# jianshu93/lash

Hardware: AMD Instinct MI355X
Metric: k-mers/s sketched (hmh, k=16) (higher is better)
Workload: dtype u64; 1 GPU; 12500 synthetic 5000000-bp genomes per GPU, -a hmh -k 16, seed 42, ASCII records resident in HBM -> sketch images in HBM (lash_sketch_batch_device: filter_out_n + k-mers + xxh3 + registers + images); genomes_per_gpu=12500, genome_length=5000000, records_per_gpu=12500, dirty=none, algo=hmh, k=16, p=0, layout=default

## Files before the change

### include/lash_gfx950.h

```cpp
#ifndef LASH_GFX950_H
#define LASH_GFX950_H
#include <stddef.h>
#include <stdint.h>

#ifdef __cplusplus
extern "C" {
#endif

#define LASH_ABI_VERSION 5

#define LASH_OK       0
#define LASH_EINVAL  (-1)
#define LASH_ENODEV  (-2)
#define LASH_EHIP    (-3)
#define LASH_ENOMEM  (-4)
#define LASH_ERANGE  (-6)
#define LASH_EFORMAT (-7)
#define LASH_ELIMIT  (-5)

#define LASH_HMH 0
#define LASH_HLL 1
#define LASH_ULL 2

#define LASH_F_HMH_X_LOW   1u
#define LASH_F_ACCUMULATE  2u
#define LASH_F_AMINO       8u
#define LASH_F_NO_DIRECT   4u

#define LASH_F_STREAM_ONLY 16u

#define LASH_F_NO_SOLE     32u

typedef struct lash_ctx lash_ctx;
typedef struct lash_packed lash_packed;

typedef struct {
    int32_t  algo;
    int32_t  k;
    int32_t  p;
    uint32_t flags;
    uint64_t seed;
} lash_params;

typedef struct {
    uint8_t base_code[4];
    uint8_t kmer_lsb_first;
    uint8_t hmh_x_low;
    uint8_t hmh_reg_be;
    uint8_t hll_bucket_high;
    char    hmh_header[8];
    char    hll_header[8];
    char    ull_header[8];
    uint8_t fastq_skip_bad;
    uint8_t aa_code_zero_based;
    uint8_t reserved[6];
} lash_layout;

typedef struct {
    float    pack_ms;
    float    sketch_ms;
    float    finalize_ms;
    uint32_t calls;
    uint32_t sketch_launches;
    uint32_t sketch_workgroups;
    uint32_t direct_launches;
    uint64_t kmers;
    uint64_t bases_last;
    uint64_t packed_bytes;
    float    direct_ms;
    uint32_t defer_launches;
    uint32_t sole_launches;
} lash_timing;

int         lash_abi_version(void);
int         lash_device_count(void);
const char *lash_strerror(int code);
int         lash_ctx_create(lash_ctx **out, int device);
void        lash_ctx_destroy(lash_ctx *ctx);
int         lash_ctx_set_stream(lash_ctx *ctx, void *hip_stream);
int         lash_ctx_synchronize(lash_ctx *ctx);
const char *lash_ctx_last_error(lash_ctx *ctx);
int         lash_ctx_enable_timing(lash_ctx *ctx, int on);
int         lash_ctx_get_timing(lash_ctx *ctx, lash_timing *out);

void       *lash_host_alloc_pinned(size_t bytes);
void        lash_host_free_pinned(void *p);

int         lash_params_check(const lash_params *prm);
size_t      lash_sketch_image_bytes(int algo, int p);

void        lash_layout_default(lash_layout *out);
int         lash_layout_check(const lash_layout *lay);
int         lash_layout_parse(const char *spec, lash_layout *out);
size_t      lash_layout_header_bytes(const lash_layout *lay, int algo);
size_t      lash_layout_image_bytes(const lash_layout *lay, int algo, int p);
int         lash_ctx_set_layout(lash_ctx *ctx, const lash_layout *lay);
int         lash_ctx_get_layout(lash_ctx *ctx, lash_layout *out);

int lash_sketch_batch(lash_ctx *ctx, const lash_params *prm,
                      const uint8_t *seq, const uint64_t *rec_off, uint64_t n_rec,
                      const uint64_t *genome_rec_off, uint32_t n_genomes, uint8_t *out_images);

int lash_sketch_batch_async(lash_ctx *ctx, const lash_params *prm,
                            const uint8_t *seq, const uint64_t *rec_off, uint64_t n_rec,
                            const uint64_t *genome_rec_off, uint32_t n_genomes, uint8_t *out_images);

int lash_sketch_batch_device(lash_ctx *ctx, const lash_params *prm,
                             const uint8_t *d_seq, const uint64_t *d_rec_off, uint64_t n_rec,
                             const uint64_t *genome_rec_off, const uint64_t *genome_byte_off,
                             uint32_t n_genomes, uint8_t *d_out_images);

#define LASH_FMT_FASTA 1
#define LASH_FMT_FASTQ 2
int lash_sketch_files_raw(lash_ctx *ctx, const lash_params *prm, const uint8_t *raw, const uint64_t *file_off,
                          const uint8_t *file_fmt, uint32_t n_files, uint8_t *out_images);
int lash_sketch_files_raw_device(lash_ctx *ctx, const lash_params *prm, const uint8_t *d_raw, const uint64_t *file_off,
                                 const uint8_t *file_fmt, uint32_t n_files, uint8_t *d_out_images);
uint32_t lash_ctx_format_errors(lash_ctx *ctx, uint32_t *file_index, uint32_t cap);

typedef struct lash_rec_index lash_rec_index;
int      lash_fasta_index(lash_ctx *ctx, const uint8_t *raw, const uint64_t *file_off, uint32_t n_files, lash_rec_index **out);
int      lash_fasta_index_device(lash_ctx *ctx, const uint8_t *d_raw, const uint64_t *file_off, uint32_t n_files, lash_rec_index **out);
uint64_t lash_rec_index_n_records(const lash_rec_index *index);
int      lash_rec_index_start(lash_ctx *ctx, const lash_rec_index *index, uint64_t *out);
int      lash_rec_index_id_len(lash_ctx *ctx, const lash_rec_index *index, uint32_t *out);
int      lash_rec_index_file(lash_ctx *ctx, const lash_rec_index *index, uint32_t *out);
void     lash_rec_index_free(lash_ctx *ctx, lash_rec_index *index);
int      lash_sketch_records_raw(lash_ctx *ctx, const lash_params *prm, const uint8_t *raw, const uint64_t *file_off, uint32_t n_files,
                                 const lash_rec_index *index, uint64_t r0, uint64_t r1, uint8_t *out_images);

typedef struct lash_win_index lash_win_index;
int      lash_fasta_windows(lash_ctx *ctx, const uint8_t *raw, const uint64_t *file_off, uint32_t n_files, const lash_rec_index *index,
                            uint64_t window, lash_win_index **out);
int      lash_fasta_windows_device(lash_ctx *ctx, const uint8_t *d_raw, const uint64_t *file_off, uint32_t n_files, const lash_rec_index *index,
                                   uint64_t window, lash_win_index **out);
uint64_t lash_win_index_n_windows(const lash_win_index *windows);
uint64_t lash_win_index_bytes(const lash_win_index *windows);
const uint8_t *lash_win_index_buffer_device(const lash_win_index *windows);
int      lash_win_index_record(lash_ctx *ctx, const lash_win_index *windows, uint64_t *out);
int      lash_win_index_begin(lash_ctx *ctx, const lash_win_index *windows, uint64_t *out);
int      lash_win_index_length(lash_ctx *ctx, const lash_win_index *windows, uint64_t *out);
int      lash_win_index_offset(lash_ctx *ctx, const lash_win_index *windows, uint64_t *out);
int      lash_sketch_windows_raw(lash_ctx *ctx, const lash_params *prm, const lash_win_index *windows, uint64_t w0, uint64_t w1,
                                 uint8_t *out_images);
void     lash_win_index_free(lash_ctx *ctx, lash_win_index *windows);

typedef struct lash_tr_index lash_tr_index;
int      lash_fasta_translate(lash_ctx *ctx, const uint8_t *raw, const uint64_t *file_off, uint32_t n_files, const lash_rec_index *index,
                              lash_tr_index **out);
int      lash_fasta_translate_device(lash_ctx *ctx, const uint8_t *d_raw, const uint64_t *file_off, uint32_t n_files, const lash_rec_index *index,
                                     lash_tr_index **out);
uint64_t lash_tr_index_n_segments(const lash_tr_index *translated);
uint64_t lash_tr_index_bytes(const lash_tr_index *translated);
const uint8_t *lash_tr_index_buffer_device(const lash_tr_index *translated);
// ... 166 lines not shown
```

### lash_amd/_lib.py

```python
import ctypes as C
import os

PKG = os.path.dirname(os.path.abspath(__file__))
LIB_PATH = os.environ.get("LASH_GFX950_LIB") or os.path.join(PKG, "liblash_gfx950.so")

OK, EINVAL, ENODEV, EHIP, ENOMEM, ELIMIT, ERANGE, EFORMAT = 0, -1, -2, -3, -4, -5, -6, -7
HMH, HLL, ULL = 0, 1, 2
F_HMH_X_LOW, F_ACCUMULATE, F_NO_DIRECT, F_AMINO, F_STREAM_ONLY, F_NO_SOLE = 1, 2, 4, 8, 16, 32
FMT_FASTA, FMT_FASTQ = 1, 2
MEASURE_JACCARD, MEASURE_CONTAIN_QUERY, MEASURE_CONTAIN_REFERENCE = 0, 1, 2
ABI_VERSION = 5


class Params(C.Structure):
    _fields_ = [("algo", C.c_int32), ("k", C.c_int32), ("p", C.c_int32), ("flags", C.c_uint32), ("seed", C.c_uint64)]


class Layout(C.Structure):
    _fields_ = [("base_code", C.c_uint8 * 4), ("kmer_lsb_first", C.c_uint8), ("hmh_x_low", C.c_uint8),
                ("hmh_reg_be", C.c_uint8), ("hll_bucket_high", C.c_uint8),
                ("hmh_header", C.c_char * 8), ("hll_header", C.c_char * 8), ("ull_header", C.c_char * 8),
                ("fastq_skip_bad", C.c_uint8), ("aa_code_zero_based", C.c_uint8), ("reserved", C.c_uint8 * 6)]


class Timing(C.Structure):
    _fields_ = [("pack_ms", C.c_float), ("sketch_ms", C.c_float), ("finalize_ms", C.c_float), ("calls", C.c_uint32),
                ("sketch_launches", C.c_uint32), ("sketch_workgroups", C.c_uint32), ("direct_launches", C.c_uint32),
                ("kmers", C.c_uint64), ("bases_last", C.c_uint64), ("packed_bytes", C.c_uint64),
                ("direct_ms", C.c_float), ("defer_launches", C.c_uint32), ("sole_launches", C.c_uint32)]


class ClusterStats(C.Structure):
    _fields_ = [("pairs", C.c_uint64), ("pruned", C.c_uint64), ("joined_on_device", C.c_uint64), ("sent_to_host", C.c_uint64),
                ("clusters", C.c_uint64)]


class DerepStats(C.Structure):
    _fields_ = [("pairs", C.c_uint64), ("pruned_not_rep", C.c_uint64), ("pruned_after_hit", C.c_uint64), ("sent_to_host", C.c_uint64),
                ("evaluated", C.c_uint64), ("representatives", C.c_uint64)]


class TreeMerge(C.Structure):
    _fields_ = [("a", C.c_uint32), ("b", C.c_uint32), ("height", C.c_double), ("size", C.c_uint32)]


class TreeStats(C.Structure):
    _fields_ = [("steps", C.c_uint64), ("rescanned_rows", C.c_uint64), ("bytes", C.c_uint64)]


class NjJoin(C.Structure):
    _fields_ = [("a", C.c_uint32), ("b", C.c_uint32), ("len_a", C.c_double), ("len_b", C.c_double)]


LINKAGE_AVERAGE, LINKAGE_SINGLE, LINKAGE_COMPLETE = 0, 1, 2

_vp, _u64, _u32, _int = C.c_void_p, C.c_uint64, C.c_uint32, C.c_int
_PP = C.POINTER(Params)
_LP = C.POINTER(Layout)

PROTOTYPES = {
    "lash_abi_version": (_int, []),
    "lash_device_count": (_int, []),
    "lash_strerror": (C.c_char_p, [_int]),
    "lash_ctx_create": (_int, [C.POINTER(_vp), _int]),
    "lash_ctx_destroy": (None, [_vp]),
    "lash_ctx_set_stream": (_int, [_vp, _vp]),
    "lash_ctx_synchronize": (_int, [_vp]),
    "lash_ctx_last_error": (C.c_char_p, [_vp]),
    "lash_ctx_enable_timing": (_int, [_vp, _int]),
    "lash_ctx_get_timing": (_int, [_vp, C.POINTER(Timing)]),
    "lash_host_alloc_pinned": (_vp, [C.c_size_t]),
    "lash_host_free_pinned": (None, [_vp]),
    "lash_params_check": (_int, [_PP]),
    "lash_sketch_image_bytes": (C.c_size_t, [_int, _int]),
    "lash_layout_default": (None, [_LP]),
    "lash_layout_check": (_int, [_LP]),
    "lash_layout_parse": (_int, [C.c_char_p, _LP]),
    "lash_layout_header_bytes": (C.c_size_t, [_LP, _int]),
    "lash_layout_image_bytes": (C.c_size_t, [_LP, _int, _int]),
    "lash_ctx_set_layout": (_int, [_vp, _LP]),
    "lash_ctx_get_layout": (_int, [_vp, _LP]),
    "lash_sketch_batch": (_int, [_vp, _PP, _vp, _vp, _u64, _vp, _u32, _vp]),
    "lash_sketch_batch_async": (_int, [_vp, _PP, _vp, _vp, _u64, _vp, _u32, _vp]),
    "lash_sketch_batch_device": (_int, [_vp, _PP, _vp, _vp, _u64, _vp, _vp, _u32, _vp]),
    "lash_sketch_files_raw": (_int, [_vp, _PP, _vp, _vp, _vp, _u32, _vp]),
    "lash_sketch_files_raw_device": (_int, [_vp, _PP, _vp, _vp, _vp, _u32, _vp]),
    "lash_ctx_format_errors": (_u32, [_vp, _vp, _u32]),
    "lash_kmer_filter_create": (_int, [_vp, _u32, _vp, C.POINTER(_vp)]),
    "lash_kmer_filter_count_raw": (_int, [_vp, _PP, _vp, _vp, _vp, _u32, _vp]),
    "lash_kmer_filter_counts": (_int, [_vp, _vp, _u32, _vp]),
    "lash_sketch_files_raw_filtered": (_int, [_vp, _PP, _vp, _vp, _vp, _u32, _vp, _u32, _vp]),
    "lash_kmer_filter_free": (None, [_vp, _vp]),
    "lash_fasta_index": (_int, [_vp, _vp, _vp, _u32, C.POINTER(_vp)]),
    "lash_fasta_index_device": (_int, [_vp, _vp, _vp, _u32, C.POINTER(_vp)]),
    "lash_rec_index_n_records": (_u64, [_vp]),
    "lash_rec_index_start": (_int, [_vp, _vp, _vp]),
    "lash_rec_index_id_len": (_int, [_vp, _vp, _vp]),
    "lash_rec_index_file": (_int, [_vp, _vp, _vp]),
    "lash_rec_index_free": (None, [_vp, _vp]),
    "lash_sketch_records_raw": (_int, [_vp, _PP, _vp, _vp, _u32, _vp, _u64, _u64, _vp]),
    "lash_fasta_windows": (_int, [_vp, _vp, _vp, _u32, _vp, _u64, C.POINTER(_vp)]),
    "lash_fasta_windows_device": (_int, [_vp, _vp, _vp, _u32, _vp, _u64, C.POINTER(_vp)]),
    "lash_win_index_n_windows": (_u64, [_vp]),
    "lash_win_index_bytes": (_u64, [_vp]),
    "lash_win_index_buffer_device": (_vp, [_vp]),
    "lash_win_index_record": (_int, [_vp, _vp, _vp]),
    "lash_win_index_begin": (_int, [_vp, _vp, _vp]),
    "lash_win_index_length": (_int, [_vp, _vp, _vp]),
    "lash_win_index_offset": (_int, [_vp, _vp, _vp]),
    "lash_sketch_windows_raw": (_int, [_vp, _PP, _vp, _u64, _u64, _vp]),
    "lash_win_index_free": (None, [_vp, _vp]),
    "lash_fasta_translate": (_int, [_vp, _vp, _vp, _u32, _vp, C.POINTER(_vp)]),
# ... 106 lines not shown
```

### lash_amd/csrc/lash_api.hip

```cpp
#include "lash_ctx.h"
#include "lash_internal.h"



namespace lashi {

size_t parse_fastx_strict(const uint8_t *d, size_t n, std::vector<uint8_t> *seq, std::vector<uint64_t> *rec_off, bool skip_bad,
                                 std::vector<std::pair<size_t, size_t>> *bad)
{
    auto line_end = [&](size_t p) { const void *q = memchr(d + p, '\n', n - p); return q ? (size_t)((const uint8_t *)q - d) : n; };
    size_t i = 0;
    if (n && d[0] == '>') {
        while (i < n) {
            i = line_end(i);
            if (i < n) ++i;
            while (i < n && d[i] != '>') {
                size_t e = line_end(i), stop = e;
                while (stop > i && d[stop - 1] == '\r') --stop;
                if (seq) seq->insert(seq->end(), d + i, d + stop);
                i = e < n ? e + 1 : n;
            }
            if (rec_off) rec_off->push_back(seq ? seq->size() : 0);
        }
        return n;
// ... 130 lines not shown
            if (val == one) { dst = 1; return true; }
            return false;
        };
        auto hdr = [&](char (&dst)[8]) {
            if (val.size() > 7) return false;
            memset(dst, 0, 8);
            memcpy(dst, val.data(), val.size());
            return true;
        };
        bool ok;
        if (key == "codes") {
            ok = val.size() == 4;
            for (size_t c = 0; ok && c < 4; ++c) {
                const char *at = strchr("ACGT", val[c]);
                if (!at || !val[c]) { ok = false; break; }
                lay.base_code[at - "ACGT"] = (uint8_t)c;
            }
        } else if (key == "kmer") ok = two("msb", "lsb", lay.kmer_lsb_first);
        else if (key == "hmh_x") ok = two("high", "low", lay.hmh_x_low);
        else if (key == "hmh_reg") ok = two("le", "be", lay.hmh_reg_be);
        else if (key == "hll_bucket") ok = two("low", "high", lay.hll_bucket_high);
        else if (key == "hmh_hdr") ok = hdr(lay.hmh_header);
        else if (key == "hll_hdr") ok = hdr(lay.hll_header);
        else if (key == "ull_hdr") ok = hdr(lay.ull_header);
        else if (key == "fastq_err") ok = two("stop", "skip", lay.fastq_skip_bad);
        else if (key == "aa_codes") ok = two("one", "zero", lay.aa_code_zero_based);
        else ok = false;
        if (!ok) return LASH_EINVAL;
    }
    if (!layout_ok(lay)) return LASH_EINVAL;
    *out = lay;
    return LASH_OK;
}

int lash_ctx_set_layout(lash_ctx *ctx, const lash_layout *lay)
{
    if (!ctx) return LASH_EINVAL;
    if (lay && !layout_ok(*lay)) return LASH_EINVAL;
    ctx->layout = lay ? *lay : kDefaultLayout;
    return LASH_OK;
}

int lash_ctx_get_layout(lash_ctx *ctx, lash_layout *out)
{
    if (!ctx || !out) return LASH_EINVAL;
    *out = ctx->layout;
    return LASH_OK;
}

int lash_ctx_create(lash_ctx **out, int device)
{
    if (!out) return LASH_EINVAL;
    *out = nullptr;
    int n = lash_device_count();
    if (n <= 0) return LASH_ENODEV;
    if (device < 0 || device >= n) return LASH_EINVAL;
    lash_ctx *ctx = new (std::nothrow) lash_ctx();
    if (!ctx) return LASH_ENOMEM;
    ctx->device = device;
    ctx->scratch.owned_by_ctx = true;
    hipDeviceProp_t prop;
    const bool ok = hipSetDevice(device) == hipSuccess && hipGetDeviceProperties(&prop, device) == hipSuccess &&
                    hipStreamCreateWithFlags(&ctx->stream, hipStreamNonBlocking) == hipSuccess;
    if (!ok) {
        lash_ctx_destroy(ctx);
        return LASH_EHIP;
    }
    ctx->own_stream = true;
    ctx->cu_count = prop.multiProcessorCount > 0 ? prop.multiProcessorCount : 256;
    *out = ctx;
    return LASH_OK;
}

void lash_ctx_destroy(lash_ctx *ctx)
{
    if (!ctx) return;
    (void)hipSetDevice(ctx->device);
    if (ctx->stream) (void)hipStreamSynchronize(ctx->stream);
    release(ctx->sole_tab);
    release(ctx->sole_brk);
    release(ctx->sole_state);
    for (DevBuf *b : {&ctx->items, &ctx->item_begin, &ctx->item_kmers, &ctx->partials, &ctx->gregs, &ctx->counter, &ctx->st_seq, &ctx->st_rec,
                      &ctx->st_img, &ctx->hll_flags, &ctx->ec_ref, &ctx->ec_qry, &ctx->ec_x, &ctx->ec_card, &ctx->wf_scratch, &ctx->wf_out, &ctx->top_buf,
                      &ctx->fa_off, &ctx->fa_scratch, &ctx->fc_scratch, &ctx->kf_keep})
        release(*b);
    {
        lash_packed &sc = ctx->scratch;
        for (DevBuf *b : {&sc.words, &sc.brk, &sc.tables, &sc.tiles, &sc.lookback, &sc.tile_begin_c, &sc.brk_bytes, &sc.fq})
            release(*b);
    }
    release(ctx->pair_ref);
    release(ctx->pair_qry);
    for (auto &s : ctx->ev_pool)
        for (auto &e : s.e)
            if (e) (void)hipEventDestroy(e);
    if (ctx->probe_host) (void)hipHostFree(ctx->probe_host);
    if (ctx->probe_ev) (void)hipEventDestroy(ctx->probe_ev);
    for (auto &sl : ctx->slot) {
        if (sl.busy && sl.d2h) (void)hipEventSynchronize(sl.d2h);
        for (DevBuf *b : {&sl.seq, &sl.rec, &sl.img}) release(*b);
        for (hipEvent_t e : {sl.h2d, sl.kern, sl.d2h}) if (e) (void)hipEventDestroy(e);
    }
    if (ctx->h2d_stream) (void)hipStreamDestroy(ctx->h2d_stream);
    if (ctx->d2h_stream) (void)hipStreamDestroy(ctx->d2h_stream);
    for (auto &hs : ctx->ring) {
        if (hs.done) (void)hipEventDestroy(hs.done);
        if (hs.ptr) (void)hipHostFree(hs.ptr);
    }
    if (ctx->own_stream && ctx->stream) (void)hipStreamDestroy(ctx->stream);
    delete ctx;
}

int lash_ctx_set_stream(lash_ctx *ctx, void *hip_stream)
{
    if (!ctx) return LASH_EINVAL;
    (void)hipSetDevice(ctx->device);
    if (ctx->stream) HIPCHK(ctx, hipStreamSynchronize(ctx->stream));
    if (ctx->own_stream && ctx->stream) (void)hipStreamDestroy(ctx->stream);
    ctx->own_stream = false;
    ctx->stream = static_cast<hipStream_t>(hip_stream);
    if (!hip_stream) {
        HIPCHK(ctx, hipStreamCreateWithFlags(&ctx->stream, hipStreamNonBlocking));
        ctx->own_stream = true;
    }
    return LASH_OK;
}

static int read_format_errors(lash_ctx *ctx)
{
    const uint32_t n = ctx->raw_files_pending;
    ctx->raw_files_pending = 0;
    ctx->bad_files.clear();
    if (!n || !ctx->scratch.d_dirty) return LASH_OK;
    std::vector<uint32_t> fl(n);
    HIPCHK(ctx, hipMemcpy(fl.data(), ctx->scratch.d_dirty + 3 * (size_t)n + 1, (size_t)n * 4, hipMemcpyDeviceToHost));
    for (uint32_t g = 0; g < n; ++g)
        if (fl[g]) ctx->bad_files.push_back(g);
    return LASH_OK;
}

static int check_pack_flag(lash_ctx *ctx, const lash_packed *pk)
{
    if (!pk || !pk->error_flag) return LASH_OK;
    uint32_t f = 0;
    HIPCHK(ctx, hipMemcpy(&f, pk->error_flag, 4, hipMemcpyDeviceToHost));
    if (f) { ctx->err = "pack kernel: look-back spin bound exceeded (results invalid)"; return LASH_EHIP; }
    return LASH_OK;
}

int lash_ctx_synchronize(lash_ctx *ctx)
{
    if (!ctx) return LASH_EINVAL;
    (void)hipSetDevice(ctx->device);
    HIPCHK(ctx, hipStreamSynchronize(ctx->stream));
    for (auto &sl : ctx->slot)
        if (sl.busy) { HIPCHK(ctx, hipEventSynchronize(sl.d2h)); sl.busy = false; }
    if (ctx->raw_files_pending) {
        const int rc = read_format_errors(ctx);
        if (rc) return rc;
        if (!ctx->bad_files.empty()) return LASH_EFORMAT;
    }
    for (const lash_packed *pk : ctx->last_packed) {
        const int rc = check_pack_flag(ctx, pk);
        if (rc) return rc;
    }
    return LASH_OK;
}

const char *lash_ctx_last_error(lash_ctx *ctx) { return ctx ? ctx->err.c_str() : ""; }

int lash_ctx_enable_timing(lash_ctx *ctx, int on)
{
    if (!ctx) return LASH_EINVAL;
    (void)hipSetDevice(ctx->device);
    HIPCHK(ctx, hipStreamSynchronize(ctx->stream));
    ctx->timing = on != 0;
    ctx->ev_used = 0;
    ctx->cur_ev = nullptr;
    ctx->last = lash_timing{};
    ctx->counter_zeroed = false;
    return LASH_OK;
}

int lash_ctx_get_timing(lash_ctx *ctx, lash_timing *out)
{
    if (!ctx || !out) return LASH_EINVAL;
    (void)hipSetDevice(ctx->device);
    HIPCHK(ctx, hipStreamSynchronize(ctx->stream));
    lash_timing t = ctx->last;
    t.pack_ms = t.sketch_ms = t.finalize_ms = t.direct_ms = 0.f;
    for (size_t i = 0; i < ctx->ev_used; ++i) {
        const EvSet &s = ctx->ev_pool[i];
        if (!s.done) continue;
        float ms = 0.f;
        if (s.pack) { HIPCHK(ctx, hipEventElapsedTime(&ms, s.e[0], s.e[1])); t.pack_ms += ms; }
        HIPCHK(ctx, hipEventElapsedTime(&ms, s.e[2], s.e[3])); t.sketch_ms += ms;
        HIPCHK(ctx, hipEventElapsedTime(&ms, s.e[3], s.e[4])); t.finalize_ms += ms;
        if (s.direct) { HIPCHK(ctx, hipEventElapsedTime(&ms, s.e[6], s.e[5])); t.direct_ms += ms; }
    }
    t.kmers = 0;
    t.bases_last = 0;
    if (ctx->counter.ptr && ctx->counter_zeroed) {
        unsigned long long c = 0;
        HIPCHK(ctx, hipMemcpy(&c, ctx->counter.ptr, 8, hipMemcpyDeviceToHost));
        t.kmers = c;
    }
    if (ctx->last_sole_only && ctx->counter.ptr && ctx->counter_zeroed) {
        unsigned long long b = 0;
        HIPCHK(ctx, hipMemcpy(&b, static_cast<const uint8_t *>(ctx->counter.ptr) + 8, 8, hipMemcpyDeviceToHost));
        t.bases_last = b;
    }
    for (const lash_packed *pk : ctx->last_packed) {
        if (!pk->n_genomes) continue;
        std::vector<uint64_t> nv(pk->n_genomes);
        HIPCHK(ctx, hipMemcpy(nv.data(), pk->d_nvalid, nv.size() * 8, hipMemcpyDeviceToHost));
        for (uint64_t v : nv) t.bases_last += v;
        if (pk->direct) {
            const uint32_t n = pk->n_genomes;
            std::vector<uint32_t> fl(5 * (size_t)n + 2);
            HIPCHK(ctx, hipMemcpy(fl.data(), pk->d_dirty, fl.size() * 4, hipMemcpyDeviceToHost));
            for (uint32_t g = 0; g < n; ++g)
                t.bases_last -= fl[g] ? fl[4 * (size_t)n + 2 + g] : fl[2 * (size_t)n + 1 + g];
        }
    }
    *out = t;
    return LASH_OK;
}

int lash_pack_device(lash_ctx *ctx, const uint8_t *d_seq, const uint64_t *d_rec_off, uint64_t n_rec,
                     const uint64_t *genome_rec_off, const uint64_t *genome_byte_off, uint32_t n_genomes,
                     lash_packed **out)
{
    if (!ctx || !out) return LASH_EINVAL;
    *out = nullptr;
    (void)hipSetDevice(ctx->device);
    lash_packed *pk = new (std::nothrow) lash_packed();
    if (!pk) return LASH_ENOMEM;
    int rc = n_genomes && (!genome_rec_off || !genome_byte_off) ? LASH_EINVAL : LASH_OK;
    if (rc == LASH_OK)
        rc = pack_into(ctx, pk, ctx->stream, nullptr, d_seq, n_genomes ? d_seq + genome_byte_off[n_genomes] : d_seq, d_rec_off, n_rec,
                       genome_rec_off, genome_byte_off, n_genomes);
    if (rc) { lash_packed_free(ctx, pk); return rc; }
    *out = pk;
    return LASH_OK;
}

void lash_packed_free(lash_ctx *ctx, lash_packed *pk)
{
    if (!pk || pk->owned_by_ctx) return;
    if (ctx) {
        (void)hipSetDevice(ctx->device);
        if (ctx->stream) (void)hipStreamSynchronize(ctx->stream);
        for (auto it = ctx->last_packed.begin(); it != ctx->last_packed.end();)
            it = (*it == pk) ? ctx->last_packed.erase(it) : it + 1;
    }
    for (DevBuf *b : {&pk->words, &pk->brk, &pk->tables, &pk->tiles, &pk->lookback, &pk->tile_begin_c, &pk->brk_bytes, &pk->fq})
        release(*b);
    delete pk;
}

uint64_t lash_packed_bytes(const lash_packed *pk)
{
    return pk ? pk->words.cap + pk->brk.cap + pk->tables.cap : 0;
}

int lash_sketch_packed_device(lash_ctx *ctx, const lash_params *prm, const lash_packed *pk, uint8_t *d_out_images)
{
    if (!ctx || !pk || (pk->n_genomes && !d_out_images)) return LASH_EINVAL;
    int rc = lash_params_check(prm);
    if (rc) return rc;
    if (prm->flags & LASH_F_AMINO) return LASH_EINVAL;
    if (pk->code_tab4 != layout_dev(ctx->layout, prm->algo).code_tab4) {
        ctx->err = "lash_sketch_packed_device: the context's layout changed its base codes / k-mer bit order since lash_pack_device";
        return LASH_EINVAL;
    }
    (void)hipSetDevice(ctx->device);
    if ((rc = timing_begin(ctx))) return rc;
    ctx->last_packed.clear();
    ctx->last_sole_only = false;
    ctx->last.calls += 1;
    return sketch_from(ctx, prm, pk, d_out_images, ctx->cur_ev);
}

int lash_sketch_batch_device(lash_ctx *ctx, const lash_params *prm, const uint8_t *d_seq, const uint64_t *d_rec_off,
                             uint64_t n_rec, const uint64_t *genome_rec_off, const uint64_t *genome_byte_off,
                             uint32_t n_genomes, uint8_t *d_out_images)
{
    if (!ctx || (n_genomes && (!d_out_images || !genome_rec_off || !genome_byte_off))) return LASH_EINVAL;
    int rc = lash_params_check(prm);
    if (rc) return rc;
    (void)hipSetDevice(ctx->device);
    ctx->last_packed.clear();
    ctx->last_sole_only = false;
    ctx->last.calls += 1;
    if (n_genomes == 0) return LASH_OK;
    if (prm->flags & LASH_F_AMINO) return sketch_aa(ctx, prm, d_seq, d_rec_off, n_rec, genome_rec_off, genome_byte_off, n_genomes, d_out_images);

    if ((rc = timing_begin(ctx))) return rc;
    EvSet *ev = ctx->cur_ev;
    TraceScope trace_scope(ctx->trace);
    TRACE("call");
    static const bool env_no_direct = getenv("LASH_NO_DIRECT") != nullptr;
    if (ctx->probe_pending && hipEventQuery(ctx->probe_ev) == hipSuccess) {
        ctx->dirty_frac = ctx->probe_tiles ? (float)ctx->probe_host[0] / (float)ctx->probe_tiles : 0.f;
        ctx->probe_pending = false;
    }
    bool direct = !(prm->flags & LASH_F_NO_DIRECT) && !env_no_direct;
    bool stream_first = false;
    if (direct && ctx->dirty_frac > 0.2f) {
        if (++ctx->direct_skipped < 8) stream_first = true;
        else ctx->direct_skipped = 0;
    }
    static const bool env_stream_first = getenv("LASH_STREAM_FIRST") != nullptr;
    ctx->scratch.stream_first = (stream_first || env_stream_first || (prm->flags & LASH_F_STREAM_ONLY)) && direct;
    ctx->last_sole_only = false;
    if (direct) {
        const SolePlan sp = make_sole_plan(prm->algo, prm->p, n_genomes, (uint32_t)ctx->cu_count);
        const uint64_t smax = sole_max_bytes(ctx, prm, sp);
        bool all_small = smax != 0 && genome_byte_off[n_genomes] >= 16, any_multi = false;
        bool identity = n_rec == n_genomes;
        for (uint32_t g = 0; g < n_genomes && all_small; ++g) {
            if (genome_byte_off[g + 1] < genome_byte_off[g] || genome_rec_off[g + 1] < genome_rec_off[g] || genome_rec_off[g + 1] > n_rec) return LASH_EINVAL;
            all_small = genome_byte_off[g + 1] - genome_byte_off[g] <= smax;
            any_multi = any_multi || genome_rec_off[g + 1] - genome_rec_off[g] > 1;
            identity = identity && genome_rec_off[g] == g && genome_rec_off[g + 1] == (uint64_t)g + 1;
        }
        if (all_small) {
            rc = sole_call(ctx, prm, sp, n_genomes, ev, [&] {
                return sole_run(ctx, prm, sp, smax, d_seq, genome_byte_off[n_genomes], d_rec_off, n_rec, any_multi, identity, genome_byte_off, nullptr,
                                n_genomes, d_out_images, nullptr);
            });
            if (rc) return rc;
            ctx->last_sole_only = true;
            ctx->cur_ev = nullptr;
            return LASH_OK;
        }
    }
    rc = pack_into(ctx, &ctx->scratch, ctx->stream, ev, d_seq, d_seq + genome_byte_off[n_genomes], d_rec_off, n_rec,
                   genome_rec_off, genome_byte_off, n_genomes, nullptr, direct);
    if (rc) return rc;
    rc = sketch_from(ctx, prm, &ctx->scratch, d_out_images, ev);
    ctx->cur_ev = nullptr;
    return rc;
}

int lash_sketch_batch_async(lash_ctx *ctx, const lash_params *prm, const uint8_t *seq, const uint64_t *rec_off, uint64_t n_rec,
                            const uint64_t *genome_rec_off, uint32_t n_genomes, uint8_t *out_images)
{
    if (!ctx || !rec_off || !genome_rec_off || (n_genomes && !out_images)) return LASH_EINVAL;
    int rc = lash_params_check(prm);
    if (rc) return rc;
    (void)hipSetDevice(ctx->device);
    for (uint64_t r = 0; r < n_rec; ++r)
        if (rec_off[r + 1] < rec_off[r]) return LASH_EINVAL;
    const uint64_t seq_bytes = rec_off[n_rec];
    if (seq_bytes && !seq) return LASH_EINVAL;
    std::vector<uint64_t> gbo(n_genomes + 1);
    for (uint32_t g = 0; g <= n_genomes; ++g) {
        if (genome_rec_off[g] > n_rec) return LASH_EINVAL;
        gbo[g] = rec_off[genome_rec_off[g]];
    }
    if (!ctx->h2d_stream) {
        HIPCHK(ctx, hipStreamCreateWithFlags(&ctx->h2d_stream, hipStreamNonBlocking));
        HIPCHK(ctx, hipStreamCreateWithFlags(&ctx->d2h_stream, hipStreamNonBlocking));
        for (auto &sl : ctx->slot)
            for (hipEvent_t *e : {&sl.h2d, &sl.kern, &sl.d2h}) HIPCHK(ctx, hipEventCreateWithFlags(e, hipEventDisableTiming));
    }
    lash_ctx::AsyncSlot &sl = ctx->slot[ctx->slot_next++ & 1u];
    if (sl.busy) { HIPCHK(ctx, hipEventSynchronize(sl.d2h)); sl.busy = false; }
    const size_t img_bytes = (size_t)n_genomes * image_bytes(ctx->layout, prm->algo, prm->p);
    auto grow = [&](DevBuf &b, size_t bytes) -> int {
        if (bytes <= b.cap) return LASH_OK;
        release(b);
        const size_t want = bytes + bytes / 8 + 256;
        HIPCHK(ctx, hipMalloc(&b.ptr, want));
        b.cap = want;
        return LASH_OK;
    };
    if ((rc = grow(sl.seq, seq_bytes + 64))) return rc;
    if ((rc = grow(sl.rec, (size_t)(n_rec + 1) * 8))) return rc;
    if ((rc = grow(sl.img, img_bytes + 64))) return rc;
    if (seq_bytes) HIPCHK(ctx, hipMemcpyAsync(sl.seq.ptr, seq, seq_bytes, hipMemcpyHostToDevice, ctx->h2d_stream));
    HIPCHK(ctx, hipMemcpyAsync(sl.rec.ptr, rec_off, (size_t)(n_rec + 1) * 8, hipMemcpyHostToDevice, ctx->h2d_stream));
    if ((prm->flags & LASH_F_ACCUMULATE) && img_bytes)
        HIPCHK(ctx, hipMemcpyAsync(sl.img.ptr, out_images, img_bytes, hipMemcpyHostToDevice, ctx->h2d_stream));
    HIPCHK(ctx, hipEventRecord(sl.h2d, ctx->h2d_stream));
    HIPCHK(ctx, hipStreamWaitEvent(ctx->stream, sl.h2d, 0));
    rc = lash_sketch_batch_device(ctx, prm, static_cast<const uint8_t *>(sl.seq.ptr), static_cast<const uint64_t *>(sl.rec.ptr), n_rec,
                                  genome_rec_off, gbo.data(), n_genomes, static_cast<uint8_t *>(sl.img.ptr));
// ... 379 lines not shown
```

### lash_amd/csrc/lash_common.h

```cpp
#pragma once
#include <stdint.h>

struct lash_hll_bias;

namespace lash {

struct GenomeDesc {
    uint64_t byte_off;
    uint64_t byte_len;
    uint64_t word_off;
    uint64_t brk_off;
    uint64_t rec_begin;
    uint64_t rec_end;
    uint32_t format;
    uint32_t handover;
};

struct WorkItem {
    uint32_t genome;
    uint32_t word_begin;
    uint32_t word_end;
    uint32_t slice;
};

constexpr uint32_t ITEM_SOLE        = 0x8000u;
constexpr int      PAD_WORDS        = 8;
constexpr int      SKETCH_WORDS_PER_THREAD = 4;
constexpr int      HMH_P            = 14;
constexpr uint32_t HMH_M            = 1u << HMH_P;

struct LayoutDev {
    uint32_t code_lo, code_hi;
    uint32_t code_tab4;
    uint32_t comp_mask;
    uint32_t hdr_bytes;
    uint32_t hmh_reg_be;
    uint32_t kmer_lsb_first;
    uint32_t hll_bucket_high;
    uint32_t aa_code_base;
    uint64_t hdr_tpl;
};

constexpr uint64_t XXH_PRIME64_1 = 0x9E3779B185EBCA87ULL;
constexpr uint64_t XXH_PRIME_MX1 = 0x165667919E3779F9ULL;
constexpr uint64_t XXH_PRIME_MX2 = 0x9FB21C651E98DF25ULL;
constexpr uint64_t XXH_SEC8  = 0x1cad21f72c81017cULL;
constexpr uint64_t XXH_SEC16 = 0xdb979083e96dd4deULL;
constexpr uint64_t XXH_SEC24 = 0x1f67b3b7a4a44072ULL;

inline uint64_t xxh3_short_seed(uint64_t seed)
{
    uint32_t lo = (uint32_t)seed;
    uint32_t sw = (lo >> 24) | ((lo >> 8) & 0xFF00u) | ((lo << 8) & 0xFF0000u) | (lo << 24);
    return seed ^ ((uint64_t)sw << 32);
}
inline uint64_t xxh3_bitflip64(uint64_t seed)  { return (XXH_SEC8 ^ XXH_SEC16) - xxh3_short_seed(seed); }
inline uint64_t xxh3_bitflip128(uint64_t seed) { return (XXH_SEC16 ^ XXH_SEC24) + xxh3_short_seed(seed); }

bool hmh_ec_closed_form(double n, double m, double *out);
double hmh_ec_from_cell_sum(double x);
double hmh_ec_cell_walk(double n, double m);
double hmh_cardinality_from_hist(const uint32_t *hist64, bool *exact);
int    hll_cardinality_from_hist(const uint32_t *hist256, int p, const lash_hll_bias *tables, double *out);
bool   dist_pair_host(int algo, int p, int k, int model, int fp32, double ref_card, double qry_card, uint32_t c_or_zero, uint32_t n_count,
                      double sum_or_union, const lash_hll_bias *tables, const double *hmh_ec, double *out, int measure = 0);

}
```

### lash_amd/csrc/lash_ctx.h

```cpp
#pragma once
#include <hip/hip_runtime.h>

#include <algorithm>
#include <chrono>
#include <cmath>
#include <cstdio>
#include <cstdlib>
#include <cstring>
#include <deque>
#include <new>
#include <string>
#include <vector>

#include "../../include/lash_gfx950.h"
#include "lash_kernels.h"
#include "ull_estimators.h"

using namespace lash;

namespace lashi {

struct DevBuf {
    void *ptr = nullptr;
    size_t cap = 0;
// ... 70 lines not shown
    const uint8_t *d_log2 = nullptr;
};

struct lash_ctx;
struct lash_sketch_set {
    int device = 0, algo = 0, p = 0;
    uint32_t n = 0;
    uint32_t hdr = 0;
    uint64_t stride = 0;
    uint32_t hmh_be = 0;
    const uint8_t *d_images = nullptr;
    DevBuf images;
    DevBuf S, T, nzcount;
    uint32_t ldT = 0, n_pad = 0;
    bool have_S = false, have_T = false, full = false;
    DevBuf lohi, bm;
    uint32_t lo = 0xFFFFFFFFu, hi = 0, bm_lo = 0, bm_band = 0;
    bool have_range = false, have_bm = false;
    std::vector<double> card;
    std::vector<uint32_t> small_idx;
    DevBuf ec_vec;
    bool have_ec_vec = false;
    DevBuf d_card, d_small;
};

int lash_set_bind(lash_ctx *ctx, lash_sketch_set *s, int algo, int p, const uint8_t *d_images, uint32_t n);
int lash_set_build_planes(lash_ctx *ctx, lash_sketch_set *s, bool want_T);
int lash_set_take_cardinalities(lash_ctx *ctx, lash_sketch_set *s, const double *card);
int lash_set_ec_vectors(lash_ctx *ctx, lash_sketch_set *qry);

struct EcBlock {
    uint32_t nrs = 0, nqs = 0, q_step = 0, rbase = 0;
    const double *X = nullptr;
};
int lash_set_ec_block(lash_ctx *ctx, const lash_sketch_set *ref, uint32_t r0, uint32_t r1, const lash_sketch_set *qry, uint32_t n_cols,
                      EcBlock &eb);
int lash_set_ec_scatter(lash_ctx *ctx, const EcBlock &eb, const lash_sketch_set *ref, uint32_t r0, const lash_sketch_set *qry, uint32_t n_cols,
                        double *out_ec);

struct PairOut {
    uint32_t *c = nullptr, *n = nullptr;
    double *u = nullptr;
};
int lash_pair_out_reserve(lash_ctx *ctx, size_t n_pairs, PairOut &d);
int lash_pair_out_fetch(lash_ctx *ctx, int algo, size_t n_pairs, const PairOut &d, uint32_t *out_c_or_zero, uint32_t *out_n,
                        double *out_sum_or_union);

struct lash_ctx {
    int device = 0;
    int cu_count = 256;
    hipStream_t stream = nullptr;
    bool own_stream = false;
    std::string err;
    lash_layout layout = kDefaultLayout;
    HostTrace trace;
    bool timing = false;
    std::deque<EvSet> ev_pool;
    size_t ev_used = 0;
    EvSet *cur_ev = nullptr;
    lash_timing last{};
    HostStage ring[32];
    unsigned ring_next = 0;
    std::vector<const lash_packed *> last_packed;
    DevBuf items, item_begin, item_kmers, partials, gregs, counter;
    uint64_t bins_budget = 0;
    int bins_slab_fill = -1; size_t bins_slab_clean = 0;
    DevBuf bins_lists, bins_meta, bins_slab;
    bool counter_zeroed = false;
    DevBuf sole_tab, sole_brk, sole_state;
    bool last_sole_only = false;
    DevBuf st_seq, st_rec, st_img;
    DevBuf kf_keep;
    DevBuf fa_off, fa_scratch;
    DevBuf fc_scratch;
    struct AsyncSlot { DevBuf seq, rec, img; hipEvent_t h2d = nullptr, kern = nullptr, d2h = nullptr; bool busy = false; };
    AsyncSlot slot[2];
    unsigned slot_next = 0;
    hipStream_t h2d_stream = nullptr, d2h_stream = nullptr;
    lash_packed scratch;
    lash_sketch_set pair_ref, pair_qry;
    DevBuf ec_ref, ec_qry, ec_x, ec_card;
    DevBuf wf_scratch, wf_out;
    DevBuf top_buf;
    DevBuf hll_flags;
    uint32_t hll_flags_n = 0;
    bool hll_flags_on_host = false;
    std::vector<uint32_t> hll_left;
    DevBuf replay_rec, replay_img;
    std::vector<uint32_t> bad_files;
    uint32_t raw_files_pending = 0;
    uint32_t *probe_host = nullptr;
    hipEvent_t probe_ev = nullptr;
    bool probe_pending = false;
    uint32_t probe_tiles = 0;
    float dirty_frac = 0.f;
    uint32_t direct_skipped = 0;
};

namespace {

int fail(lash_ctx *ctx, int code, const char *what, hipError_t e)
{
    if (ctx) {
        char buf[512];
        snprintf(buf, sizeof buf, "%s: %s", what, hipGetErrorString(e));
        ctx->err = buf;
    }
    return code;
}

#define TRACE(what) ctx->trace.mark(what)
struct TraceScope {
    HostTrace &t;
    explicit TraceScope(HostTrace &tr) : t(tr) { t.begin(); }
    ~TraceScope() { t.end(); }
};

#define HIPCHK(ctx, expr)                                              \
    do {                                                               \
        hipError_t e__ = (expr);                                       \
        if (e__ != hipSuccess) return fail((ctx), e__ == hipErrorOutOfMemory ? LASH_ENOMEM : LASH_EHIP, #expr, e__); \
    } while (0)

int reserve(lash_ctx *ctx, DevBuf &b, size_t bytes)
{
    if (bytes <= b.cap) return LASH_OK;
    if (b.ptr) {
        HIPCHK(ctx, hipStreamSynchronize(ctx->stream));
        HIPCHK(ctx, hipFree(b.ptr));
        b.ptr = nullptr;
        b.cap = 0;
    }
    size_t want = bytes + bytes / 8 + 256;
    HIPCHK(ctx, hipMalloc(&b.ptr, want));
    b.cap = want;
    return LASH_OK;
}

void release(DevBuf &b)
{
    if (b.ptr) (void)hipFree(b.ptr);
    b.ptr = nullptr;
    b.cap = 0;
}

void release(lash_sketch_set &s)
{
    for (DevBuf *b : {&s.images, &s.S, &s.T, &s.nzcount, &s.lohi, &s.bm, &s.ec_vec, &s.d_card, &s.d_small}) release(*b);
}

int upload(lash_ctx *ctx, void *d_dst, const void *h_src, size_t bytes, hipStream_t stream = nullptr)
{
    if (bytes == 0) return LASH_OK;
    if (!stream) stream = ctx->stream;
    HostStage &hs = ctx->ring[ctx->ring_next++ % 32];
    if (hs.pending) { HIPCHK(ctx, hipEventSynchronize(hs.done)); hs.pending = false; }
    if (!hs.done) HIPCHK(ctx, hipEventCreateWithFlags(&hs.done, hipEventDisableTiming));
    if (hs.cap < bytes) {
        if (hs.ptr) HIPCHK(ctx, hipHostFree(hs.ptr));
        hs.ptr = nullptr;
        hs.cap = 0;
        HIPCHK(ctx, hipHostMalloc(&hs.ptr, bytes + bytes / 4 + 4096, hipHostMallocDefault));
        hs.cap = bytes + bytes / 4 + 4096;
    }
    memcpy(hs.ptr, h_src, bytes);
    HIPCHK(ctx, hipMemcpyAsync(d_dst, hs.ptr, bytes, hipMemcpyHostToDevice, stream));
    HIPCHK(ctx, hipEventRecord(hs.done, stream));
    hs.pending = true;
    return LASH_OK;
}

struct Section { const void *src; size_t bytes; size_t off; };
size_t layout_sections(std::vector<Section> &sec)
{
    size_t at = 0;
    for (Section &x : sec) { x.off = at; at += (x.bytes + 255) & ~(size_t)255; }
    return at;
}
int upload_sections(lash_ctx *ctx, void *d_base, const std::vector<Section> &sec, size_t total, hipStream_t stream)
// ... 118 lines not shown
```

### lash_amd/csrc/lash_hll_replay.hip

```cpp
#include "lash_ctx.h"
#include "lash_internal.h"

namespace lashi {

double grid_sum(const uint8_t *regs, size_t m, int p)
{
    uint32_t hist[72] = {0};
    for (size_t i = 0; i < m; ++i) ++hist[regs[i] < 71 ? regs[i] : 71];
    double s = 0.0;
    for (int r = 0; r <= 53 - p; ++r) s += (double)hist[r] * ldexp(1.0, -r);
    return s;
}
int hll_sum_field_offset(const lash_layout &lay)
{
    const char *t = header_tpl(lay, LASH_HLL);
    int at = 0;
    for (int i = 0; i < 8 && t[i]; ++i) {
        switch (t[i]) {
        case 's': return at;
        case 'a': case 'z': case 'Q': case 'l': at += 8; break;
        case 'Z': case 'P': case 'L': at += 4; break;
        case 'p': at += 1; break;
        default: break;
        }
    }
    return -1;
}

struct ReplayRestore {
    lash_ctx *c;
    lash_timing last; bool timing; std::vector<const lash_packed *> packed; float dirty_frac; uint32_t direct_skipped; bool sole_only;
    explicit ReplayRestore(lash_ctx *x) : c(x), last(x->last), timing(x->timing), packed(x->last_packed), dirty_frac(x->dirty_frac),
                                          direct_skipped(x->direct_skipped), sole_only(x->last_sole_only) {}
    ~ReplayRestore()
    {
        c->last = last; c->timing = timing; c->last_packed = packed; c->dirty_frac = dirty_frac; c->direct_skipped = direct_skipped;
        c->last_sole_only = sole_only;
        c->probe_pending = false;
    }
};

int hll_replay_one(lash_ctx *ctx, const lash_params *prm, const uint8_t *d_seq, const std::vector<uint64_t> &rec, const uint8_t *fin,
                          const uint8_t *base, double &S, double &G, bool &carry)
{
    const int p = prm->p;
    const size_t hdr = header_bytes(ctx->layout, LASH_HLL), m = (size_t)1 << p, ib = hdr + m;
    int rc;
    if ((rc = reserve(ctx, ctx->replay_img, ib + 64))) return rc;
    if ((rc = reserve(ctx, ctx->replay_rec, (rec.size() + 1) * 8))) return rc;
    auto prefix = [&](uint64_t cut, std::vector<uint8_t> &out) -> int {
        size_t i = (size_t)(std::upper_bound(rec.begin(), rec.end(), cut) - rec.begin());
        if (i == 0) i = 1;
        std::vector<uint64_t> pr(rec.begin(), rec.begin() + i);
        if (pr.back() < cut) pr.push_back(cut);
        const uint64_t n = pr.size() - 1, goff[2] = {0, n}, gbo[2] = {pr.front(), pr.back()};
        HIPCHK(ctx, hipMemcpy(ctx->replay_rec.ptr, pr.data(), pr.size() * 8, hipMemcpyHostToDevice));
        int r = lash_sketch_batch_device(ctx, prm, d_seq, static_cast<const uint64_t *>(ctx->replay_rec.ptr), n, goff, gbo, 1,
                                         static_cast<uint8_t *>(ctx->replay_img.ptr));
        if (r) return r;
        HIPCHK(ctx, hipStreamSynchronize(ctx->stream));
        out.resize(ib);
        HIPCHK(ctx, hipMemcpy(out.data(), ctx->replay_img.ptr, ib, hipMemcpyDeviceToHost));
        if (base) for (size_t j = 0; j < m; ++j) out[hdr + j] = std::max(out[hdr + j], base[j]);
        return LASH_OK;
    };
    struct Event { uint64_t cut; uint32_t j; uint8_t neu, old; std::vector<uint8_t> before; };
    std::vector<Event> events;
    std::vector<std::pair<uint32_t, uint8_t>> todo;
    for (size_t j = 0; j < m; ++j)
        if (fin[hdr + j] > 53 - p && (!base || fin[hdr + j] != base[j])) todo.push_back({(uint32_t)j, fin[hdr + j]});
    std::vector<uint8_t> probe;
    while (!todo.empty()) {
        const auto [j, val] = todo.back();
        todo.pop_back();
        uint64_t lo = rec.front(), hi = rec.back();
        while (hi - lo > 1) {
            const uint64_t mid = lo + (hi - lo) / 2;
            if ((rc = prefix(mid, probe))) return rc;
            if (probe[hdr + j] >= val) hi = mid; else lo = mid;
        }
        Event e;
        e.cut = hi; e.j = j; e.neu = val;
        if ((rc = prefix(hi - 1, e.before))) return rc;
        e.old = e.before[hdr + j];
        if (e.old > 53 - p && (!base || e.old != base[j])) todo.push_back({j, e.old});
        events.push_back(std::move(e));
    }
    if (events.empty()) {
        if (carry) { S += grid_sum(fin + hdr, m, p) - G; }
        else memcpy(&S, fin + hll_sum_field_offset(ctx->layout), 8);
        G = grid_sum(fin + hdr, m, p);
        return LASH_OK;
    }
    std::sort(events.begin(), events.end(), [](const Event &a, const Event &b) { return a.cut < b.cut; });
    if (carry) S += grid_sum(events[0].before.data() + hdr, m, p) - G;
    else S = grid_sum(events[0].before.data() + hdr, m, p);
    double grid_after = 0.0;
    for (size_t i = 0; i < events.size(); ++i) {
        const Event &e = events[i];
        if (i) S += grid_sum(e.before.data() + hdr, m, p) - grid_after;
        S -= ldexp(1.0, -(int)e.old) - ldexp(1.0, -(int)e.neu);
        std::vector<uint8_t> after(e.before.begin() + hdr, e.before.end());
        after[e.j] = e.neu;
        grid_after = grid_sum(after.data(), m, p);
    }
    G = grid_sum(fin + hdr, m, p);
    S += G - grid_after;
    carry = true;
    return LASH_OK;
}

int hll_replay_sums(lash_ctx *ctx, const lash_params *prm0, const uint8_t *d_seq, const uint64_t *d_rec_off, const uint64_t *h_rec_off,
                           const uint64_t *genome_rec_off, uint8_t *d_images, uint8_t *h_images, const std::vector<uint32_t> &flagged,
                           std::vector<uint32_t> &left)
{
    left.clear();
    if (flagged.empty()) return LASH_OK;
    const int p = prm0->p, sum_at = hll_sum_field_offset(ctx->layout);
    const size_t hdr = header_bytes(ctx->layout, LASH_HLL), m = (size_t)1 << p, ib = hdr + m;
// ... 124 lines not shown
```

### lash_amd/csrc/lash_internal.h

```cpp
#pragma once
#include <functional>
#include <utility>
#include <vector>

#include "lash_ctx.h"

namespace lashi {

int pack_into(lash_ctx *ctx, lash_packed *pk, hipStream_t stream, EvSet *ev, const uint8_t *d_seq, const uint8_t *d_seq_end,
              const uint64_t *d_rec_off, uint64_t n_rec, const uint64_t *genome_rec_off, const uint64_t *genome_byte_off,
              uint32_t n_genomes, const uint8_t *formats = nullptr, bool direct = false);
int probe_dirty(lash_ctx *ctx, lash_packed *pk, hipStream_t stream);
uint64_t sole_max_bytes(const lash_ctx *ctx, const lash_params *prm, const SolePlan &sp);
int sole_run(lash_ctx *ctx, const lash_params *prm, const SolePlan &sp, uint64_t max_len, const uint8_t *d_seq, uint64_t seq_bytes,
             const uint64_t *d_rec_off, uint64_t n_rec, bool any_multi, bool rec_identity, const uint64_t *genome_byte_off, const lash_packed *pk,
             uint32_t n_genomes, uint8_t *d_out_images, uint32_t *per_genome_ndel);
int sole_call(lash_ctx *ctx, const lash_params *prm, const SolePlan &sp, uint32_t n_genomes, EvSet *ev, const std::function<int()> &run);
int sketch_from(lash_ctx *ctx, const lash_params *prm, const lash_packed *pk, uint8_t *d_out_images, EvSet *ev, bool allow_bins = true,
                const uint32_t *d_keep = nullptr);
int sketch_aa(lash_ctx *ctx, const lash_params *prm, const uint8_t *d_seq, const uint64_t *d_rec_off, uint64_t n_rec,
              const uint64_t *genome_rec_off, const uint64_t *genome_byte_off, uint32_t n_genomes, uint8_t *d_out_images, bool allow_bins = true);

double grid_sum(const uint8_t *regs, size_t m, int p);
int hll_sum_field_offset(const lash_layout &lay);
int hll_replay_one(lash_ctx *ctx, const lash_params *prm, const uint8_t *d_seq, const std::vector<uint64_t> &rec, const uint8_t *fin,
                   const uint8_t *base, double &S, double &G, bool &carry);
int hll_replay_sums(lash_ctx *ctx, const lash_params *prm0, const uint8_t *d_seq, const uint64_t *d_rec_off, const uint64_t *h_rec_off,
                    const uint64_t *genome_rec_off, uint8_t *d_images, uint8_t *h_images, const std::vector<uint32_t> &flagged,
                    std::vector<uint32_t> &left);
std::vector<uint32_t> hll_flagged(lash_ctx *ctx);

int files_raw_staged(lash_ctx *ctx, const lash_params *prm, const uint8_t *raw, const uint8_t *d_raw, const uint64_t *file_off,
                     const uint8_t *file_fmt, uint32_t n_files, uint8_t *out_images);
size_t parse_fastx_strict(const uint8_t *d, size_t n, std::vector<uint8_t> *seq, std::vector<uint64_t> *rec_off, bool skip_bad = false,
                          std::vector<std::pair<size_t, size_t>> *bad = nullptr);

}
```

### lash_amd/csrc/lash_kernels.h

```cpp
#pragma once
#include <hip/hip_runtime.h>
#include <stdint.h>

#include "lash_common.h"

namespace lash {

struct BinGenome { uint64_t list_off; uint32_t cap; uint32_t pad; };
struct SketchArgs {
    const uint32_t   *words;
    const uint32_t   *brk;
    const uint32_t   *zero_words;
    const GenomeDesc *genomes;
    const uint64_t   *nvalid;
    const WorkItem   *items;
    const uint32_t   *item_order;
    uint8_t          *partials;
    uint32_t         *gregs;
    uint32_t         *item_kmers;
    uint8_t          *images;
    uint64_t          image_bytes;
    uint64_t          alpha_bits;
    int               accumulate;
    const uint8_t    *seq;
    union {
        const uint32_t *brk_bytes;
        const uint32_t *keep;
    };
    const uint8_t    *safe;
    uint32_t         *dirty;
    uint32_t         *nslow;
    uint32_t         *ndel;
    uint32_t         *ndel2;
    const uint64_t   *rec_off;
    const uint32_t   *nonuniform;
    uint32_t         *hll_corner;
    uint64_t          bitflip;
    LayoutDev         lay;
    uint32_t          partial_stride;
    uint32_t          stage_off;
    uint32_t          stage_stride;
    uint32_t          sigq_depth;
    uint32_t          nreg32;
    int               k;
    int               p;
    uint32_t          item_base;
    unsigned long long *item_trace;
    uint32_t         *bin_lists;
    uint32_t         *bin_cnt;
    uint32_t         *bin_slab;
    uint32_t         *bin_spill;
    const BinGenome  *bin_genomes;
    uint32_t          bins, bin_shift, bin_S, bin_sub_shift;
    uint32_t          bin_flush_words;
    uint32_t          bin_lds_off, bin_wave_bytes;
    uint32_t          bin_slab_words;
    uint32_t          bin_genome0;
};

struct SketchPlan {
    int      algo, k, p;
    bool     variant;
    bool     use_lds;
    uint32_t threads;
    uint32_t lds_bytes;
    uint32_t nreg32;
    uint32_t partial_bytes;
    uint32_t partial_stride;
    bool     defer = false;
    uint32_t sigq_depth = 7;
    bool     bins = false;
    bool     bytes = false;
    uint32_t bins_log2 = 0, bin_shift = 0, bin_S = 0, bin_sub_shift = 0, bin_flush_words = 1;
};
uint32_t sketch_bin_wave_bytes(const SketchPlan &plan);
struct BinApplyArgs {
    const uint32_t *lists, *cnt;
    uint32_t *spill;
    uint32_t *slab;
    const BinGenome *genomes;
    uint8_t  *partials;
    uint32_t *item_kmers;
    const uint32_t *genome_item_begin;
    const WorkItem *items;
    const uint64_t *nvalid;
    int       k;
    uint64_t  partial_stride;
    uint32_t  virt0, genome0;
    uint32_t  bins, bin_shift, slab_words;
    int       algo, p;
    uint8_t  *images;
    uint64_t  image_bytes;
    uint64_t  hdr_tpl;
    uint32_t  hdr_bytes;
    unsigned long long *kmer_counter;
};
hipError_t launch_bins_apply(const BinApplyArgs &args, uint32_t n_group_genomes, hipStream_t stream);

SketchPlan make_sketch_plan(int algo, int k, int p, bool variant, bool small_items = false, bool allow_bins = true);
hipError_t launch_sketch_stream(const SketchPlan &plan, const SketchArgs &args, uint32_t n_items, hipStream_t stream);
uint32_t sketch_direct_stage_bytes(const SketchPlan &plan);
hipError_t launch_sketch(const SketchPlan &plan, const SketchArgs &args, uint32_t n_items, hipStream_t stream,
                         bool direct = false);
hipError_t launch_sketch_keep(const SketchPlan &plan, const SketchArgs &args, uint32_t n_items, hipStream_t stream);
inline bool sketch_plan_keeps(const SketchPlan &plan) { return plan.use_lds && !plan.bins && !plan.bytes; }

struct KmerFilterArgs {
    const uint32_t   *words;
    const uint32_t   *brk;
    const GenomeDesc *genomes;
    const uint64_t   *nvalid;
    const uint64_t   *cell_word;
    const uint8_t    *log2_cells;
    uint32_t         *cells;
    uint32_t         *keep;
    uint32_t          comp_mask;
    uint32_t          n_genomes;
    uint32_t          min_count;
    int               k;
};
constexpr uint64_t KMER_FILTER_MUL1 = 0x9E3779B97F4A7C15ull, KMER_FILTER_MUL2 = 0xC2B2AE3D27D4EB4Full;
hipError_t launch_kmer_count(const KmerFilterArgs &args, uint64_t max_bytes, hipStream_t stream);
hipError_t launch_kmer_keep(const KmerFilterArgs &args, uint64_t max_bytes, hipStream_t stream);
struct SoleArgs {
    const uint8_t  *seq;
    uint64_t        seq_bytes;
    const uint64_t *genome_byte_off;
    const uint32_t *brk_abs;
    const uint8_t  *safe;
    uint32_t       *ndel;
    const uint32_t   *words;
    const uint32_t   *brk;
    const GenomeDesc *genomes;
    const uint64_t   *nvalid;
    const uint32_t *chunk_begin;
    uint32_t        n_chunks;
    uint32_t       *ticket;
    uint64_t        max_len;
    uint8_t        *images;
    uint64_t        image_bytes;
// ... 179 lines not shown
```

### lash_amd/csrc/lash_plan.hip

```cpp
#include "lash_ctx.h"
#include "lash_internal.h"
#include "text_tiles.h"

namespace lashi {


int pack_into(lash_ctx *ctx, lash_packed *pk, hipStream_t stream, EvSet *ev, const uint8_t *d_seq, const uint8_t *d_seq_end,
              const uint64_t *d_rec_off, uint64_t n_rec, const uint64_t *genome_rec_off, const uint64_t *genome_byte_off,
              uint32_t n_genomes, const uint8_t *formats, bool direct)
{
    if (n_genomes && (!genome_byte_off || (!formats && !genome_rec_off))) return LASH_EINVAL;
    pk->error_flag = nullptr;
    pk->direct = direct && !formats && n_genomes;
    direct = pk->direct;
    pk->d_seq = d_seq;
    std::vector<GenomeDesc> &descs = pk->h_descs;
    descs.assign(n_genomes, GenomeDesc{});
    pk->byte_len.assign(n_genomes, 0);
    uint64_t wo = 0, bo = 0;
    for (uint32_t g = 0; g < n_genomes; ++g) {
        if (genome_byte_off[g + 1] < genome_byte_off[g]) return LASH_EINVAL;
        if (!formats && (genome_rec_off[g + 1] < genome_rec_off[g] || genome_rec_off[g + 1] > n_rec)) return LASH_EINVAL;
        if (formats && formats[g] != LASH_FMT_FASTA && formats[g] != LASH_FMT_FASTQ) return LASH_EINVAL;
        GenomeDesc &d = descs[g];
// ... 45 lines not shown
        any_multi = descs[g].format != 0u || descs[g].rec_end - descs[g].rec_begin > 1;
    pk->any_multi = any_multi;
    pk->d_rec_off = d_rec_off;
    pk->n_rec = n_rec;
    pk->h_nvalid.assign(n_genomes + 1, 0);
    if (direct) std::copy(pk->byte_len.begin(), pk->byte_len.end(), pk->h_nvalid.begin());
    if (ev) { ev->pack = true; HIPCHK(ctx, hipEventRecord(ev->e[0], stream)); }
    if (!direct) {
        std::vector<Section> sec = {{descs.data(), descs.size() * sizeof(GenomeDesc), 0},
                                    {tile_begin.data(), tile_begin.size() * 4, 0},
                                    {pk->h_nvalid.data(), pk->h_nvalid.size() * 8, 0}};
        const size_t total = layout_sections(sec);
        if ((rc = reserve(ctx, pk->tables, total))) return rc;
        if ((rc = upload_sections(ctx, pk->tables.ptr, sec, total, stream))) return rc;
        uint8_t *tb = static_cast<uint8_t *>(pk->tables.ptr);
        pk->d_descs = reinterpret_cast<GenomeDesc *>(tb + sec[0].off);
        pk->d_tile_begin = reinterpret_cast<uint32_t *>(tb + sec[1].off);
        pk->d_nvalid = reinterpret_cast<uint64_t *>(tb + sec[2].off);
        TRACE("pack: tables uploaded");
        if (any_multi) HIPCHK(ctx, hipMemsetAsync(pk->brk.ptr, 0, pk->total_brk * 4, stream));
        HIPCHK(ctx, hipMemsetAsync(pk->lookback.ptr, 0, lb_bytes + (formats ? (size_t)(5 * (size_t)n_genomes + 2) * 4 : 0), stream));
        TRACE("pack: memsets queued");
    } else {
        pk->d_descs = nullptr; pk->d_tile_begin = nullptr; pk->d_nvalid = nullptr;
        if (any_multi && (rc = reserve(ctx, pk->brk_bytes, pk->total_brk * 4))) return rc;
    }
    PackArgs pa{};
    pa.seq = d_seq;
    pa.seq_end = d_seq_end;
    pa.rec_off = d_rec_off;
    pa.genomes = pk->d_descs;
    pa.words = static_cast<uint32_t *>(pk->words.ptr);
    pa.brk = static_cast<uint32_t *>(pk->brk.ptr);
    pa.nvalid = pk->d_nvalid;
    pa.code_tab4 = layout_dev(ctx->layout, LASH_HMH).code_tab4;
    pk->code_tab4 = pa.code_tab4;
    pa.file_err = formats ? pk->d_dirty + 3 * (size_t)n_genomes + 1 : nullptr;
    uint64_t *lb = static_cast<uint64_t *>(pk->lookback.ptr);
    PackV2Args v2{};
    v2.tiles = static_cast<const TileInfo *>(pk->tiles.ptr);
    v2.desc = lb;
    v2.error_flag = reinterpret_cast<uint32_t *>(lb + n_tiles);
    v2.desc2 = reinterpret_cast<uint32_t *>(lb + n_tiles + 1);
    v2.ticket = reinterpret_cast<uint32_t *>((reinterpret_cast<uintptr_t>(v2.desc2 + n_tiles + 1) + 127) & ~(uintptr_t)127);
    v2.n_tiles = (uint32_t)n_tiles;
    PackMapArgs pm{};
    pm.seq = d_seq;
    pm.rec_off = d_rec_off;
    pm.genomes = pa.genomes;
    pm.tile_begin = pk->d_tile_begin;
    pm.tiles = static_cast<TileInfo *>(pk->tiles.ptr);
    pm.n_tiles = (uint32_t)n_tiles;
    pm.n_genomes = n_genomes;
    pk->error_flag = direct ? nullptr : v2.error_flag;
    if (!direct) {
        HIPCHK(ctx, launch_pack_v2(pa, v2, pm, (uint32_t)ctx->cu_count, formats != nullptr, stream));
        if (formats) {
            std::vector<FqFile> fq;
            uint64_t blocks = 0;
            const uint64_t bb = TEXT_TILE;
            for (uint32_t g = 0; g < n_genomes; ++g) {
                if (formats[g] != LASH_FMT_FASTQ || descs[g].byte_len == 0) continue;
                const uint64_t nb = (descs[g].byte_len + bb - 1) / bb;
                fq.push_back(FqFile{descs[g].byte_off, descs[g].byte_len, (uint32_t)blocks, (uint32_t)nb, g, 0u});
                blocks += nb;
            }
            if (blocks > 0x7FFFFFFFull) return LASH_ELIMIT;
            if (!fq.empty()) {
                std::vector<Section> sec = {{fq.data(), fq.size() * sizeof(FqFile), 0}};
                const size_t total = layout_sections(sec), tab = total;
                if ((rc = reserve(ctx, pk->fq, tab + fastq_check_scratch_words((uint32_t)fq.size(), (uint32_t)blocks) * 4))) return rc;
                if ((rc = upload_sections(ctx, pk->fq.ptr, sec, total, stream))) return rc;
                uint8_t *fb = static_cast<uint8_t *>(pk->fq.ptr);
                HIPCHK(ctx, launch_fastq_check(d_seq, reinterpret_cast<const FqFile *>(fb + sec[0].off), (uint32_t)fq.size(), (uint32_t)blocks,
                                               reinterpret_cast<uint32_t *>(fb + tab), pa.file_err, stream));
            }
        }
    }
    if (ev) HIPCHK(ctx, hipEventRecord(ev->e[1], stream));
    TRACE("pack: done");
    return LASH_OK;
}

int probe_dirty(lash_ctx *ctx, lash_packed *pk, hipStream_t stream)
{
    uint32_t *tbc = static_cast<uint32_t *>(pk->tile_begin_c.ptr);
    HIPCHK(ctx, launch_dirty_tile_scan(pk->d_tile_begin, pk->d_dirty, pk->n_genomes, tbc, tbc + pk->n_genomes + 1, stream));
    if (!ctx->probe_host) {
        HIPCHK(ctx, hipHostMalloc(reinterpret_cast<void **>(&ctx->probe_host), 64, hipHostMallocDefault));
        ctx->probe_host[0] = 0;
        HIPCHK(ctx, hipEventCreateWithFlags(&ctx->probe_ev, hipEventDisableTiming));
    }
    if (!ctx->probe_pending) {
        HIPCHK(ctx, hipMemcpyAsync(ctx->probe_host, tbc + pk->n_genomes + 1, 4, hipMemcpyDeviceToHost, stream));
        HIPCHK(ctx, hipEventRecord(ctx->probe_ev, stream));
        ctx->probe_pending = true;
        ctx->probe_tiles = pk->h_tile_begin.empty() ? 0 : pk->h_tile_begin.back();
    }
    return LASH_OK;
}

uint64_t bins_budget_bytes(lash_ctx *ctx)
{
    if (const char *e = getenv("LASH_BINS_MB")) return (uint64_t)std::max(64, atoi(e)) << 20;
    if (!ctx->bins_budget) {
        size_t free_b = 0, total_b = 0;
        uint64_t b = 6144ull << 20;
        if (hipMemGetInfo(&free_b, &total_b) == hipSuccess && total_b)
            b = std::max<uint64_t>(1ull << 30, std::min<uint64_t>({24ull << 30, (uint64_t)total_b / 12, (uint64_t)free_b / 3}));
        else (void)hipGetLastError();
        ctx->bins_budget = b;
    }
    return ctx->bins_budget;
}

struct BinsRun {
    std::vector<uint32_t> group_end;
    std::vector<BinGenome> table;
    const BinGenome *d_table = nullptr;
    uint32_t *d_cnt = nullptr, *d_spill = nullptr;
    WorkItem *d_vitems = nullptr;
    uint32_t *d_vbegin = nullptr;
    uint32_t slab_words = 0, max_group = 0;
    bool fits = true;
};
static int bins_prepare(lash_ctx *ctx, const SketchPlan &plan, const std::vector<uint64_t> &entries_of_genome, uint32_t n_genomes, BinsRun &br)
{
    const uint32_t B = 1u << plan.bins_log2;
    br.slab_words = plan.nreg32;
    const uint64_t budget = bins_budget_bytes(ctx);
    br.table.resize(n_genomes);
    uint64_t bytes = 0, off = 0, group_max_bytes = 0;
    uint32_t in_group = 0;
    for (uint32_t g = 0; g < n_genomes; ++g) {
        const uint64_t m_row = std::max<uint64_t>(1, 1024u >> (plan.bins_log2 + plan.bin_sub_shift));
        uint64_t mean = entries_of_genome[g] / B * (2 * m_row + 6) / (2 * m_row) * 2 / 3 + 4;
        uint64_t sq = 1; while (sq * sq < mean) ++sq;
        const uint64_t cap = (mean + mean / 8 + 8 * sq + 1024 + 63) & ~63ull;
        if (cap > 0xFFFFFFFFull) { br.fits = false; return LASH_OK; }
        const uint64_t mine = B * cap * 4 + (uint64_t)br.slab_words * 4;
        if (mine > budget) { br.fits = false; return LASH_OK; }
        if (in_group && (bytes + mine > budget || in_group == 65535u)) {
            br.group_end.push_back(g);
            br.max_group = std::max(br.max_group, in_group);
            bytes = 0; off = 0; in_group = 0;
        }
        br.table[g] = BinGenome{off, (uint32_t)cap, 0u};
        off += B * cap;
        bytes += mine;
        group_max_bytes = std::max(group_max_bytes, off * 4);
        ++in_group;
    }
    br.group_end.push_back(n_genomes);
    br.max_group = std::max(br.max_group, in_group);
    int rc;
    if ((rc = reserve(ctx, ctx->bins_lists, group_max_bytes + 256))) return rc;
    {
        void *before = ctx->bins_slab.ptr;
        if ((rc = reserve(ctx, ctx->bins_slab, (size_t)br.max_group * br.slab_words * 4 + 256))) return rc;
        if (ctx->bins_slab.ptr != before) ctx->bins_slab_fill = -1;
    }
    std::vector<WorkItem> vitems(n_genomes);
    std::vector<uint32_t> vbegin(n_genomes + 1);
    for (uint32_t g = 0; g < n_genomes; ++g) { vitems[g] = WorkItem{g, 0u, 4u, 0u}; vbegin[g] = g; }
    vbegin[n_genomes] = n_genomes;
    std::vector<Section> sec = {{br.table.data(), br.table.size() * sizeof(BinGenome), 0}, {vitems.data(), vitems.size() * sizeof(WorkItem), 0},
                                {vbegin.data(), vbegin.size() * 4, 0}};
    const size_t tabs = layout_sections(sec), cnt_bytes = ((size_t)br.max_group * B * 4 + 255) & ~(size_t)255, spill_bytes = cnt_bytes;
    if ((rc = reserve(ctx, ctx->bins_meta, tabs + cnt_bytes + spill_bytes + 256))) return rc;
    if ((rc = upload_sections(ctx, ctx->bins_meta.ptr, sec, tabs, ctx->stream))) return rc;
    uint8_t *mb = static_cast<uint8_t *>(ctx->bins_meta.ptr);
    br.d_table = reinterpret_cast<const BinGenome *>(mb + sec[0].off);
    br.d_vitems = reinterpret_cast<WorkItem *>(mb + sec[1].off);
    br.d_vbegin = reinterpret_cast<uint32_t *>(mb + sec[2].off);
    br.d_cnt = reinterpret_cast<uint32_t *>(mb + tabs);
    br.d_spill = reinterpret_cast<uint32_t *>(mb + tabs + cnt_bytes);
    return LASH_OK;
}
static bool bins_write_images(const lash_params *prm) { return prm->algo == LASH_ULL && !(prm->flags & LASH_F_ACCUMULATE); }
static size_t bins_partials(const SketchPlan &plan, const lash_params *prm, size_t n_items, size_t n_genomes)
{
    if (!plan.bins) return n_items + 1;
// ... 158 lines not shown
        off_tmp.resize((size_t)n_genomes + 1);
        off_tmp[0] = 0;
        for (uint32_t g = 0; g < n_genomes; ++g) off_tmp[g + 1] = off_tmp[g] + pk->byte_len[g];
        off = off_tmp.data();
    }
    {
        const uint64_t fixed = image_bytes / 4 + 256;
        const uint64_t total = off[n_genomes] - off[0] + fixed * n_genomes;
        const uint64_t min_cost = 512ull * sp.threads;
        const uint64_t by_cost = std::max<uint64_t>(n_wg, total / min_cost);
        sole_chunks(off, n_genomes, fixed, (uint32_t)std::min<uint64_t>((uint64_t)n_wg * sole_chunks_per_wg(), by_cost), chunk_begin);
    }
    const uint32_t n_chunks = (uint32_t)chunk_begin.size() - 1;
    int rc;
    std::vector<Section> sec = {{chunk_begin.data(), chunk_begin.size() * 4, 0}};
    const bool gbo_is_rec_off = !packed && !any_multi && n_rec == n_genomes && d_rec_off != nullptr && rec_identity;
    if (!packed && !gbo_is_rec_off) sec.push_back({genome_byte_off, ((size_t)n_genomes + 1) * 8, 0});
    const size_t tabs = layout_sections(sec), counts_bytes = ((size_t)n_wg * 16 + 255) & ~(size_t)255;
    if ((rc = reserve(ctx, ctx->sole_tab, tabs + counts_bytes + 256))) return rc;
    if ((rc = upload_sections(ctx, ctx->sole_tab.ptr, sec, tabs, ctx->stream))) return rc;
    uint8_t *tb = static_cast<uint8_t *>(ctx->sole_tab.ptr);
    if (!ctx->sole_state.ptr) {
        if ((rc = reserve(ctx, ctx->sole_state, 256))) return rc;
        HIPCHK(ctx, hipMemsetAsync(ctx->sole_state.ptr, 0, 256, ctx->stream));
    }
    if ((rc = reserve(ctx, ctx->counter, 256))) return rc;
    if (!ctx->counter_zeroed) {
        HIPCHK(ctx, hipMemsetAsync(ctx->counter.ptr, 0, 256, ctx->stream));
        ctx->counter_zeroed = true;
    }
    SoleArgs sa{};
    sa.chunk_begin = reinterpret_cast<const uint32_t *>(tb + sec[0].off);
    sa.n_chunks = n_chunks;
    sa.ticket = static_cast<uint32_t *>(ctx->sole_state.ptr);
    sa.wg_counts = reinterpret_cast<unsigned long long *>(tb + tabs);
    sa.max_len = max_len;
    sa.safe = static_cast<const uint8_t *>(ctx->counter.ptr) + 128;
    if (!packed) {
        sa.seq = d_seq;
        sa.seq_bytes = seq_bytes;
        sa.genome_byte_off = gbo_is_rec_off ? d_rec_off : reinterpret_cast<const uint64_t *>(tb + sec[1].off);
        sa.ndel = per_genome_ndel;
        if (any_multi) {
            const size_t bm_bytes = ((seq_bytes + 63) / 32 + 2) * 4 + 2048;
            if ((rc = reserve(ctx, ctx->sole_brk, bm_bytes))) return rc;
            HIPCHK(ctx, hipMemsetAsync(ctx->sole_brk.ptr, 0, bm_bytes, ctx->stream));
            HIPCHK(ctx, launch_sole_mark(d_rec_off, n_rec, seq_bytes, static_cast<uint32_t *>(ctx->sole_brk.ptr), ctx->stream));
            sa.brk_abs = static_cast<const uint32_t *>(ctx->sole_brk.ptr);
        }
    } else {
        sa.words = static_cast<const uint32_t *>(pk->words.ptr);
        sa.brk = static_cast<const uint32_t *>(pk->brk.ptr);
        sa.genomes = pk->d_descs;
        sa.nvalid = pk->d_nvalid;
    }
    image_fields(sa, ctx, prm, d_out_images);
    sa.bitflip = prm->algo == LASH_HMH ? xxh3_bitflip128(prm->seed) : xxh3_bitflip64(prm->seed);
    sa.nreg32 = prm->algo == LASH_HMH ? HMH_M : prm->algo == LASH_HLL ? (1u << prm->p) : (2u << prm->p);
    HIPCHK(ctx, launch_sole(sp, prm->algo, prm->k, x_low, packed, sa, n_wg, ctx->stream));
    unsigned long long *ctr = static_cast<unsigned long long *>(ctx->counter.ptr);
    HIPCHK(ctx, launch_sole_census(sa.wg_counts, n_wg, ctr, ctr + 1, sa.ticket, ctx->stream));
    ctx->last.sole_launches += 1;
    return LASH_OK;
}

int sole_call(lash_ctx *ctx, const lash_params *prm, const SolePlan &sp, uint32_t n_genomes, EvSet *ev, const std::function<int()> &run)
{
    int rc;
    if ((rc = arm_hll_flags(ctx, prm, n_genomes, false))) return rc;
    if (ev) HIPCHK(ctx, hipEventRecord(ev->e[2], ctx->stream));
    if ((rc = run())) return rc;
    if (ev) { HIPCHK(ctx, hipEventRecord(ev->e[3], ctx->stream)); HIPCHK(ctx, hipEventRecord(ev->e[4], ctx->stream)); ev->done = true; }
    ctx->last.sketch_launches += 1;
    ctx->last.sketch_workgroups = (uint32_t)std::min<uint64_t>((uint64_t)ctx->cu_count * sp.wg_per_cu, n_genomes);
    return LASH_OK;
}


struct PlanKnobs {
    uint64_t slice_factor, item_cap_words;
    uint32_t tail_split;
    bool tail_geo;
    int64_t defer_min;
};
static PlanKnobs plan_knobs()
{
    static const uint64_t slice_factor = getenv("LASH_SLICE_FACTOR") ? std::max(1, atoi(getenv("LASH_SLICE_FACTOR"))) : 0;
    static const uint64_t item_cap = getenv("LASH_ITEM_CAP_WORDS") ? std::max(1024, atoi(getenv("LASH_ITEM_CAP_WORDS"))) : 0;
    static const uint32_t tail_split = getenv("LASH_TAIL_SPLIT") ? (uint32_t)std::max(1, atoi(getenv("LASH_TAIL_SPLIT"))) : 0u;
    const char *dm_env = getenv("LASH_DEFER_MIN");
    return PlanKnobs{slice_factor, item_cap, tail_split, !(getenv("LASH_TAIL_GEO") && atoi(getenv("LASH_TAIL_GEO")) == 0),
                     dm_env ? atoll(dm_env) : 600000};
}

static bool may_defer(const SketchPlan &plan) { return plan.algo == LASH_HMH && plan.use_lds; }

struct ItemPlan {
    std::vector<WorkItem> items;
    std::vector<uint32_t> item_begin;
    uint32_t max_slices = 0;
    bool all_sole = false;
    std::vector<uint32_t> order;
    std::vector<uint32_t> handover;
    uint64_t n_coarse = 0;
    uint64_t total_words = 0;
    bool defer = false;
};

static ItemPlan plan_items(const std::vector<uint64_t> &blen, const SketchPlan &plan, uint64_t slots, bool direct, bool stream_first,
                           const PlanKnobs &knobs)
{
    const uint32_t n_genomes = (uint32_t)blen.size();
    const bool defer_eligible = may_defer(plan);
    ItemPlan ip;
    for (uint64_t b : blen) ip.total_words += (b + 15) / 16;
    const uint64_t step = (uint64_t)plan.threads * SKETCH_WORDS_PER_THREAD;
    const uint64_t min_slice = step * 8;
    uint64_t len_lo = ~0ull, len_hi = 0;
    for (uint64_t b : blen) { len_lo = std::min(len_lo, b); len_hi = std::max(len_hi, b); }
    const bool equal_genomes = n_genomes > 0 && len_hi <= len_lo + len_lo / 4;
    const uint64_t slice_factor = knobs.slice_factor ? knobs.slice_factor : (defer_eligible ? (equal_genomes ? 1 : 2) : 4);
    uint64_t target = ip.total_words / (slots * slice_factor) + 1;
    if (!plan.use_lds) target = ip.total_words / std::max<uint64_t>(1, slots / 4) + 1;
    target = std::max(target, min_slice);
    {
        const uint64_t cap = knobs.item_cap_words ? knobs.item_cap_words : (defer_eligible ? 131072 : 65536);
        bool any_cut = false;
        for (uint64_t b : blen) any_cut = any_cut || (((b + 15) / 16 + 3) & ~3ull) > target;
        if (any_cut && !equal_genomes) target = std::max(min_slice, std::min(target, cap));
    }
    ip.all_sole = plan.use_lds && !plan.bins && n_genomes > 0;
    ip.item_begin.assign(n_genomes + 1, 0);
    ip.items.reserve(n_genomes * 2);
    auto slicing = [&](uint32_t g, uint64_t &nw, uint64_t &ns, uint64_t &per) {
        nw = ((blen[g] + 15) / 16 + 3) & ~3ull;
        ns = nw ? (nw + target - 1) / target : 0;
        per = nw ? (((nw + ns - 1) / ns) + 3) & ~3ull : 0;
    };
    const uint32_t tail_split = knobs.tail_split ? knobs.tail_split : (direct && stream_first ? 1u : (defer_eligible && equal_genomes ? 2u : 4u));
    const uint64_t tail_min = min_slice / 8;
    uint64_t fine_from = ~0ull;
    uint64_t c_lo = ~0ull, c_hi = 0;
    for (uint32_t g = 0; g < n_genomes; ++g) {
        uint64_t nw, ns, per;
        slicing(g, nw, ns, per);
        if (!nw) continue;
        const uint64_t cnt = (nw + per - 1) / per, last = nw - (cnt - 1) * per;
        ip.n_coarse += cnt;
        c_lo = std::min(c_lo, last); c_hi = std::max(c_hi, cnt > 1 ? per : last);
    }
    const bool unequal = c_hi > c_lo + c_lo / 4;
    if (plan.use_lds && tail_split > 1 && ip.n_coarse > slots && !unequal) fine_from = ip.n_coarse - slots;
    uint64_t ci = 0;
    for (uint32_t g = 0; g < n_genomes; ++g) {
        ip.item_begin[g] = (uint32_t)ip.items.size();
        uint64_t nw, ns, per;
        slicing(g, nw, ns, per);
        if (nw == 0) { ip.all_sole = false; continue; }
        uint32_t s = 0;
        const bool whole = ns == 1 && plan.use_lds && !plan.bins;
        for (uint64_t b = 0; b < nw; b += per, ++ci) {
            const uint64_t e = std::min(nw, b + per);
            uint64_t sub = e - b;
            if (ci >= fine_from) {
                uint64_t split = tail_split;
                const uint64_t from_end = ip.n_coarse - 1 - ci;
                if (knobs.tail_geo && from_end < slots / 2) split *= 2;
                if (knobs.tail_geo && from_end < slots / 4) split *= 2;
                while (split > 1 && (e - b) / split < tail_min) split /= 2;
                if (split > 1) sub = ((((e - b) + split - 1) / split) + 3) & ~3ull;
            }
            const bool sole = whole && sub == e - b;
            for (uint64_t bb = b; bb < e; bb += sub, ++s)
                ip.items.push_back(WorkItem{g, (uint32_t)bb, (uint32_t)std::min(e, bb + sub), (s & 0x7FFFu) | (sole ? ITEM_SOLE : 0u)});
        }
        ip.max_slices = std::max<uint32_t>(ip.max_slices, s);
        if (s != 1) ip.all_sole = false;
    }
    ip.item_begin[n_genomes] = (uint32_t)ip.items.size();
    const uint32_t n_items = (uint32_t)ip.items.size();
    if (direct) {
        ip.handover.resize(n_genomes);
        for (uint32_t g = 0; g < n_genomes; ++g)
            ip.handover[g] = std::max<uint32_t>(1u, (ip.item_begin[g + 1] - ip.item_begin[g]) * (plan.threads / 64u) / 32u);
    }
    if (n_items > slots && unequal && !plan.bins && plan.use_lds) {
        auto bucket = [&](uint32_t n) {
            const uint32_t e = 31u - (uint32_t)__builtin_clz(n | 1u);
            const uint32_t m = e >= 3 ? (n >> (e - 3)) & 7u : 0u;
            return 255u - (e * 8u + m);
        };
        uint32_t count[257] = {0};
        for (const WorkItem &w : ip.items) ++count[bucket(w.word_end - w.word_begin) + 1];
        for (int b = 0; b < 256; ++b) count[b + 1] += count[b];
        ip.order.resize(n_items);
        for (uint32_t i = 0; i < n_items; ++i) ip.order[count[bucket(ip.items[i].word_end - ip.items[i].word_begin)]++] = i;
    }
    ip.defer = defer_eligible && ip.n_coarse > 0 && knobs.defer_min >= 0 && ip.total_words * 16 / ip.n_coarse >= (uint64_t)knobs.defer_min;
    return ip;
}

static SketchPlan choose_plan(lash_ctx *ctx, const lash_params *prm, bool small_items, bool allow_bins, uint64_t largest_hbm)
{
    const bool x_low = rule_variant(ctx->layout, prm->algo, prm->flags);
    SketchPlan plan = make_sketch_plan(prm->algo, prm->k, prm->p, x_low, small_items, allow_bins);
    if (plan.bins && largest_hbm + (uint64_t)plan.nreg32 * 4 + (64u << 20) > bins_budget_bytes(ctx))
        plan = make_sketch_plan(prm->algo, prm->k, prm->p, x_low, small_items, false);
    return plan;
}

static int reserve_stage(lash_ctx *ctx, const lash_params *prm, const SketchPlan &plan, const ItemPlan &ip, const std::vector<uint64_t> &entries,
                         BinsRun &br)
{
    const size_t n_items = ip.items.size(), n_genomes = ip.item_begin.size() - 1;
    const size_t n_virtual = plan.bins ? n_genomes : 0;
    int rc;
    if ((rc = reserve(ctx, ctx->partials, bins_partials(plan, prm, n_items, n_genomes) * plan.partial_stride))) return rc;
    if ((rc = reserve(ctx, ctx->item_kmers, (n_items + n_virtual + 1) * 4))) return rc;
    if ((rc = reserve(ctx, ctx->counter, 256))) return rc;
    return plan.bins ? bins_prepare(ctx, plan, entries, (uint32_t)n_genomes, br) : LASH_OK;
}

static SketchArgs sketch_args(const lash_ctx *ctx, const lash_params *prm, const SketchPlan &plan, const WorkItem *d_items, uint8_t *images)
{
    SketchArgs sa{};
    image_fields(sa, ctx, prm, images);
    sa.bitflip = prm->algo == LASH_HMH ? xxh3_bitflip128(prm->seed) : xxh3_bitflip64(prm->seed);
    sa.items = d_items;
    sa.partials = static_cast<uint8_t *>(ctx->partials.ptr);
    sa.gregs = static_cast<uint32_t *>(ctx->gregs.ptr);
    sa.item_kmers = static_cast<uint32_t *>(ctx->item_kmers.ptr);
    sa.partial_stride = plan.partial_stride;
    sa.nreg32 = plan.nreg32;
    return sa;
}

static int finalize_run(lash_ctx *ctx, const lash_params *prm, const SketchPlan &plan, const BinsRun &br, const ItemPlan &ip, FinalizeArgs fa,
                        uint32_t group_above, uint8_t *images)
{
    const uint32_t n_items = (uint32_t)ip.items.size(), n_genomes = (uint32_t)ip.item_begin.size() - 1;
    uint32_t max_slices = ip.max_slices;
    image_fields(fa, ctx, prm, images);
    fa.partials = static_cast<const uint8_t *>(ctx->partials.ptr);
    fa.item_kmers = static_cast<const uint32_t *>(ctx->item_kmers.ptr);
    if (plan.bins) {
        fa.item_kmers += n_items;
        fa.items = br.d_vitems;
        fa.genome_item_begin = br.d_vbegin;
        max_slices = 1;
    }
    fa.kmer_counter = static_cast<unsigned long long *>(ctx->counter.ptr);
    fa.partial_stride = plan.partial_stride;
    fa.partial_base_off = 0;
    fa.algo = prm->algo;
    fa.src_images = 0;
    fa.group = 0;
    if (max_slices > group_above && n_genomes <= 65535u)
        for (fa.group = 32u; (max_slices + fa.group - 1) / fa.group > 16u; fa.group *= 32u) {}
    if (plan.bins && bins_write_images(prm)) {
    } else if (ip.all_sole) {
        HIPCHK(ctx, launch_census(fa, n_genomes, ctx->stream));
    } else {
        HIPCHK(ctx, launch_reduce_groups(fa, n_genomes, max_slices, ctx->stream));
        HIPCHK(ctx, launch_finalize(fa, n_genomes, ctx->stream));
    }
    return LASH_OK;
}

static int item_trace_begin(lash_ctx *ctx, uint32_t n_items, SketchArgs &sa)
{
    if (!getenv("LASH_ITEM_TRACE") || !n_items) return LASH_OK;
    HIPCHK(ctx, hipMalloc(&sa.item_trace, (size_t)n_items * 32));
    HIPCHK(ctx, hipMemsetAsync(sa.item_trace, 0, (size_t)n_items * 32, ctx->stream));
    return LASH_OK;
}
static int item_trace_end(lash_ctx *ctx, const ItemPlan &ip, uint32_t threads, SketchArgs &sa)
{
    if (!sa.item_trace) return LASH_OK;
    const uint32_t n_items = (uint32_t)ip.items.size();
    std::vector<unsigned long long> h((size_t)n_items * 4);
    HIPCHK(ctx, hipStreamSynchronize(ctx->stream));
    HIPCHK(ctx, hipMemcpy(h.data(), sa.item_trace, h.size() * 8, hipMemcpyDeviceToHost));
    (void)hipFree(sa.item_trace);
    sa.item_trace = nullptr;
    if (FILE *f = fopen(getenv("LASH_ITEM_TRACE"), "a")) {
        fprintf(f, "# launch: %u items, %u threads, order %s; columns: slot item genome word_begin word_end start_10ns end_10ns hw_id xcc_id\n",
                n_items, threads, ip.order.empty() ? "item" : "longest first");
        for (uint32_t b = 0; b < n_items; ++b) {
            const uint32_t i = ip.order.empty() ? b : ip.order[b];
            const WorkItem &w = ip.items[i];
            fprintf(f, "%u %u %u %u %u %llu %llu %u %u\n", b, i, w.genome, w.word_begin, w.word_end, h[4ull * i], h[4ull * i + 1],
                    (unsigned)(h[4ull * i + 2] & 0xFFFFFFFFu), (unsigned)(h[4ull * i + 2] >> 32));
        }
        fclose(f);
    }
    return LASH_OK;
}

static int sole_batch(lash_ctx *ctx, const lash_params *prm, const SolePlan &sp, uint64_t sole_max, const lash_packed *pk, uint8_t *images,
                      uint32_t *ndel)
{
    const uint32_t n = pk->n_genomes;
    if (!pk->direct) return sole_run(ctx, prm, sp, sole_max, nullptr, 0, nullptr, 0, false, false, nullptr, pk, n, images, nullptr);
    std::vector<uint64_t> gbo((size_t)n + 1);
    for (uint32_t g = 0; g < n; ++g) gbo[g] = pk->h_descs[g].byte_off;
    gbo[n] = pk->h_descs[n - 1].byte_off + pk->h_descs[n - 1].byte_len;
    bool identity = pk->n_rec == n;
    for (uint32_t g = 0; g < n && identity; ++g) identity = pk->h_descs[g].rec_begin == g && pk->h_descs[g].rec_end == g + 1u;
    return sole_run(ctx, prm, sp, sole_max, pk->d_seq, gbo[n], pk->d_rec_off, pk->n_rec, pk->any_multi, identity, gbo.data(), nullptr, n, images, ndel);
}

static int direct_launches(lash_ctx *ctx, const lash_params *prm, const SketchPlan &plan, lash_packed *pk, const ItemPlan &ip, SketchArgs &sa,
                           const BinsRun &br, const uint32_t *d_item_begin, EvSet *ev)
{
    const uint32_t n_items = (uint32_t)ip.items.size(), n_genomes = pk->n_genomes;
    const bool ranged = plan.bins || !plan.use_lds, direct_pass = !pk->stream_first, timed = ev && (ranged || direct_pass);
    sa.seq = pk->d_seq;
    sa.brk_bytes = static_cast<const uint32_t *>(pk->brk_bytes.ptr);
    sa.dirty = pk->d_dirty;
    sa.rec_off = pk->d_rec_off;
    sa.nonuniform = pk->d_dirty + 3 * (size_t)n_genomes + 1;
    sa.nslow = pk->d_dirty + n_genomes + 1;
    sa.ndel = sa.nslow + n_genomes;
    sa.ndel2 = pk->d_dirty + 4 * (size_t)n_genomes + 2;
    int rc;
    if (pk->stream_first)
        HIPCHK(ctx, hipMemsetAsync(pk->d_dirty, 0x01, (size_t)n_genomes * 4, ctx->stream));
    if (direct_pass && !ranged && (rc = item_trace_begin(ctx, n_items, sa))) return rc;
    if (timed) HIPCHK(ctx, hipEventRecord(ev->e[6], ctx->stream));
    rc = launch_items(ctx, plan, prm, sa, br, ip.item_begin, d_item_begin, [&](const SketchArgs &a, uint32_t cnt) -> int {
        if (direct_pass) HIPCHK(ctx, launch_sketch(plan, a, cnt, ctx->stream, true));
        if (ranged) HIPCHK(ctx, launch_sketch_stream(plan, a, cnt, ctx->stream));
        return LASH_OK;
    });
    if (rc) return rc;
    if (timed) { HIPCHK(ctx, hipEventRecord(ev->e[5], ctx->stream)); ev->direct = true; }
    if ((rc = item_trace_end(ctx, ip, plan.threads, sa))) return rc;
    if (direct_pass) {
        if ((rc = probe_dirty(ctx, pk, ctx->stream))) return rc;
        ctx->last.direct_launches += n_items ? 1 : 0;
        ctx->last.defer_launches += (n_items && plan.defer) ? 1 : 0;
    }
    if (!ranged) HIPCHK(ctx, launch_sketch_stream(plan, sa, n_items, ctx->stream));
    return LASH_OK;
}

int sketch_from(lash_ctx *ctx, const lash_params *prm, const lash_packed *pk, uint8_t *d_out_images, EvSet *ev, bool allow_bins,
                const uint32_t *d_keep)
{
    if (d_keep && (pk->direct || !(prm->flags & LASH_F_NO_SOLE))) return LASH_EINVAL;
    const uint32_t n_genomes = pk->n_genomes;
    lash_packed *mpk = const_cast<lash_packed *>(pk);
    const SolePlan sole_plan = make_sole_plan(prm->algo, prm->p, n_genomes, (uint32_t)ctx->cu_count);
    uint64_t sole_max = sole_max_bytes(ctx, prm, sole_plan);
    if (pk->direct && n_genomes && pk->h_descs[n_genomes - 1].byte_off + pk->h_descs[n_genomes - 1].byte_len < 16) sole_max = 0;
    std::vector<uint64_t> blen(n_genomes);
    uint32_t n_sole = 0;
    uint64_t total_bytes = 0, largest = 0;
    for (uint32_t g = 0; g < n_genomes; ++g) {
        const bool sole = sole_max && pk->byte_len[g] <= sole_max;
        blen[g] = sole ? 0 : pk->byte_len[g];
        n_sole += sole;
        total_bytes += blen[g];
        largest = std::max<uint64_t>(largest, pk->byte_len[g]);
    }
    int rc;
    if (n_sole == n_genomes && n_genomes && !pk->direct) {
        if ((rc = sole_call(ctx, prm, sole_plan, n_genomes, ev, [&] { return sole_batch(ctx, prm, sole_plan, sole_max, pk, d_out_images, nullptr); })))
            return rc;
        ctx->last_packed.push_back(pk);
        return LASH_OK;
    }
    const bool small_items = n_genomes > n_sole && total_bytes / (n_genomes - n_sole) < 100000u;
    SketchPlan plan = choose_plan(ctx, prm, small_items, allow_bins, largest * 5);
    const uint32_t lds_wg = plan.lds_bytes + ((pk->direct || may_defer(plan) || plan.bytes) ? sketch_direct_stage_bytes(plan) : 0u);
    const uint32_t wg_per_cu = plan.use_lds ? std::max(1u, (160u * 1024u) / std::max(lds_wg, 1u)) : 4u;
    const uint64_t slots = (uint64_t)ctx->cu_count * std::min(wg_per_cu, 2048u / plan.threads);
    const ItemPlan ip = plan_items(blen, plan, slots, pk->direct, pk->stream_first, plan_knobs());
    const uint32_t n_items = (uint32_t)ip.items.size();
    plan.defer = ip.defer && !d_keep;
    if (d_keep && !sketch_plan_keeps(plan)) return LASH_EINVAL;
    if (pk->direct)
        for (uint32_t g = 0; g < n_genomes; ++g) mpk->h_descs[g].handover = ip.handover[g];
    TRACE("sketch: planned");

    std::vector<uint64_t> entries;
    if (plan.bins) {
        entries.assign(n_genomes, 0);
        const uint64_t tile_words = (uint64_t)plan.threads * SKETCH_WORDS_PER_THREAD;
        for (const WorkItem &w : ip.items) entries[w.genome] += ((w.word_end - w.word_begin + tile_words - 1) / tile_words) * tile_words * 16;
    }
    BinsRun br;
    if ((rc = reserve_stage(ctx, prm, plan, ip, entries, br))) return rc;
    if (!br.fits) return sketch_from(ctx, prm, pk, d_out_images, ev, false, d_keep);
    const WorkItem *d_items;
    const uint32_t *d_item_begin, *d_item_order = nullptr;
    {
        std::vector<Section> sec = {{ip.items.data(), (size_t)n_items * sizeof(WorkItem), 0},
                                    {ip.item_begin.data(), (size_t)(n_genomes + 1) * 4, 0}};
        if (pk->direct) {
            sec.push_back({pk->h_descs.data(), pk->h_descs.size() * sizeof(GenomeDesc), 0});
            sec.push_back({pk->h_tile_begin.data(), pk->h_tile_begin.size() * 4, 0});
            sec.push_back({pk->h_nvalid.data(), pk->h_nvalid.size() * 8, 0});
        }
        const size_t order_sec = sec.size();
        if (!ip.order.empty()) sec.push_back({ip.order.data(), ip.order.size() * 4, 0});
        const size_t total = layout_sections(sec);
        DevBuf &dst = pk->direct ? mpk->tables : ctx->items;
        if ((rc = reserve(ctx, dst, total + 256))) return rc;
        if ((rc = upload_sections(ctx, dst.ptr, sec, total, ctx->stream))) return rc;
        if (ev) HIPCHK(ctx, hipEventRecord(ev->e[2], ctx->stream));
        uint8_t *tb = static_cast<uint8_t *>(dst.ptr);
        d_items = reinterpret_cast<const WorkItem *>(tb + sec[0].off);
        d_item_begin = reinterpret_cast<const uint32_t *>(tb + sec[1].off);
        d_item_order = ip.order.empty() ? nullptr : reinterpret_cast<const uint32_t *>(tb + sec[order_sec].off);
        if (pk->direct) {
            mpk->d_descs = reinterpret_cast<GenomeDesc *>(tb + sec[2].off);
            mpk->d_tile_begin = reinterpret_cast<uint32_t *>(tb + sec[3].off);
            mpk->d_nvalid = reinterpret_cast<uint64_t *>(tb + sec[4].off);
            HIPCHK(ctx, hipMemsetAsync(pk->d_dirty, 0, (size_t)(5 * (size_t)n_genomes + 2) * 4, ctx->stream));
            if (pk->any_multi) {
                uint32_t *nonuni = pk->d_dirty + 3 * (size_t)n_genomes + 1;
                HIPCHK(ctx, launch_rec_uniform(pk->d_descs, pk->d_rec_off, n_genomes, pk->n_rec, nonuni, ctx->stream));
                HIPCHK(ctx, launch_brk_bytes(pk->d_descs, pk->d_rec_off, n_genomes, pk->n_rec, nonuni, static_cast<uint32_t *>(pk->brk_bytes.ptr),
                                             ctx->stream));
            }
        }
    }
    if (!ctx->counter_zeroed) {
        HIPCHK(ctx, hipMemsetAsync(ctx->counter.ptr, 0, 256, ctx->stream));
        ctx->counter_zeroed = true;
    }
    TRACE("sketch: items uploaded");

    if ((rc = arm_hll_flags(ctx, prm, n_genomes, true))) return rc;
    SketchArgs sa = sketch_args(ctx, prm, plan, d_items, d_out_images);
    sa.words = static_cast<const uint32_t *>(pk->words.ptr);
    sa.brk = static_cast<const uint32_t *>(pk->brk.ptr);
    sa.zero_words = reinterpret_cast<const uint32_t *>(static_cast<const uint8_t *>(ctx->counter.ptr) + 16);
    sa.genomes = pk->d_descs;
    sa.nvalid = pk->d_nvalid;
    sa.item_order = d_item_order;
    sa.safe = static_cast<const uint8_t *>(ctx->counter.ptr) + 128;
    if (d_keep) sa.keep = d_keep;
    if (pk->direct) {
        if ((rc = direct_launches(ctx, prm, plan, mpk, ip, sa, br, d_item_begin, ev))) return rc;
    } else {
        rc = launch_items(ctx, plan, prm, sa, br, ip.item_begin, d_item_begin, [&](const SketchArgs &a, uint32_t cnt) -> int {
            HIPCHK(ctx, d_keep ? launch_sketch_keep(plan, a, cnt, ctx->stream) : launch_sketch(plan, a, cnt, ctx->stream));
            return LASH_OK;
        });
        if (rc) return rc;
        ctx->last.defer_launches += (n_items && plan.defer) ? 1 : 0;
    }
    if (n_sole && (rc = sole_batch(ctx, prm, sole_plan, sole_max, pk, d_out_images, pk->stream_first ? sa.ndel2 : sa.ndel))) return rc;
    if (ev) HIPCHK(ctx, hipEventRecord(ev->e[3], ctx->stream));
    TRACE("sketch: launched");

    FinalizeArgs fa{};
    fa.items = d_items;
    fa.genome_item_begin = d_item_begin;
    fa.nvalid = pk->d_nvalid;
    fa.descs = n_sole ? pk->d_descs : nullptr;
    fa.skip_max_len = n_sole ? sole_max : 0;
    if ((rc = finalize_run(ctx, prm, plan, br, ip, fa, n_genomes <= 4096u ? 8u : 32u, d_out_images))) return rc;
    if (ev) { HIPCHK(ctx, hipEventRecord(ev->e[4], ctx->stream)); ev->done = true; }
    TRACE("finalize: launched");
    ctx->last_packed.push_back(pk);
    ctx->last.sketch_launches += n_items ? 1 : 0;
    ctx->last.sketch_workgroups = n_items;
    for (uint32_t g = 0; g < n_genomes; ++g)
        ctx->last.packed_bytes += (pk->byte_len[g] + 15) / 16 * 4 + (pk->byte_len[g] + 31) / 32 * 4;
    return LASH_OK;
}

int sketch_aa(lash_ctx *ctx, const lash_params *prm, const uint8_t *d_seq, const uint64_t *d_rec_off, uint64_t n_rec,
              const uint64_t *genome_rec_off, const uint64_t *genome_byte_off, uint32_t n_genomes, uint8_t *d_out_images, bool allow_bins)
{
    int rc;
    if (allow_bins && (rc = timing_begin(ctx))) return rc;
    EvSet *ev = ctx->cur_ev;
    uint64_t largest = 0;
    for (uint32_t g = 0; g < n_genomes; ++g)
        largest = std::max<uint64_t>(largest, (genome_byte_off[g + 1] - genome_byte_off[g]) + 32 * (genome_rec_off[g + 1] - genome_rec_off[g]));
    const SketchPlan plan = choose_plan(ctx, prm, false, allow_bins, largest * 6);
    std::vector<GenomeDesc> descs(n_genomes, GenomeDesc{});
    ItemPlan ip;
    ip.item_begin.assign(n_genomes + 1, 0);
    for (uint32_t g = 0; g < n_genomes; ++g) {
        if (genome_rec_off[g + 1] < genome_rec_off[g] || genome_rec_off[g + 1] > n_rec) return LASH_EINVAL;
        GenomeDesc &d = descs[g];
        d.byte_off = genome_byte_off[g];
        d.byte_len = genome_byte_off[g + 1] - genome_byte_off[g];
        d.rec_begin = genome_rec_off[g];
        d.rec_end = genome_rec_off[g + 1];
        ip.item_begin[g] = (uint32_t)ip.items.size();
        const uint64_t nr = d.rec_end - d.rec_begin;
        if (nr > 0xFFFFFFFFull) return LASH_ELIMIT;
        uint32_t s = 0;
        for (uint64_t r0 = 0; r0 < nr; r0 += AA_RECORDS_PER_ITEM, ++s)
            ip.items.push_back(WorkItem{g, (uint32_t)r0, (uint32_t)std::min<uint64_t>(nr, r0 + AA_RECORDS_PER_ITEM), s & 0x7FFFu});
        ip.max_slices = std::max(ip.max_slices, s);
    }
    ip.item_begin[n_genomes] = (uint32_t)ip.items.size();
    const uint32_t n_items = (uint32_t)ip.items.size();
    std::vector<uint64_t> entries;
    if (plan.bins) {
        entries.resize(n_genomes);
        for (uint32_t g = 0; g < n_genomes; ++g) {
            const uint64_t e = descs[g].byte_len + 32 * (descs[g].rec_end - descs[g].rec_begin);
            entries[g] = e + e / 4 + (uint64_t)plan.threads * 256;
        }
    }
    BinsRun br;
    if ((rc = reserve_stage(ctx, prm, plan, ip, entries, br))) return rc;
    if (!br.fits) return sketch_aa(ctx, prm, d_seq, d_rec_off, n_rec, genome_rec_off, genome_byte_off, n_genomes, d_out_images, false);
    std::vector<Section> sec = {{ip.items.data(), (size_t)n_items * sizeof(WorkItem), 0}, {ip.item_begin.data(), (size_t)(n_genomes + 1) * 4, 0},
                                {descs.data(), descs.size() * sizeof(GenomeDesc), 0}};
    const size_t total = layout_sections(sec);
    if ((rc = reserve(ctx, ctx->items, total + 256))) return rc;
    if ((rc = upload_sections(ctx, ctx->items.ptr, sec, total, ctx->stream))) return rc;
    uint8_t *tb = static_cast<uint8_t *>(ctx->items.ptr);
    const uint32_t *d_item_begin = reinterpret_cast<const uint32_t *>(tb + sec[1].off);
    if (!ctx->counter_zeroed) {
        HIPCHK(ctx, hipMemsetAsync(ctx->counter.ptr, 0, 256, ctx->stream));
        ctx->counter_zeroed = true;
    }
    if (ev) HIPCHK(ctx, hipEventRecord(ev->e[2], ctx->stream));
    if ((rc = arm_hll_flags(ctx, prm, n_genomes, true))) return rc;
    SketchArgs sa = sketch_args(ctx, prm, plan, reinterpret_cast<const WorkItem *>(tb + sec[0].off), d_out_images);
    sa.seq = d_seq;
    sa.rec_off = d_rec_off;
    sa.genomes = reinterpret_cast<const GenomeDesc *>(tb + sec[2].off);
    rc = launch_items(ctx, plan, prm, sa, br, ip.item_begin, d_item_begin, [&](const SketchArgs &a, uint32_t cnt) -> int {
        HIPCHK(ctx, launch_sketch_aa(plan, a, cnt, ctx->stream));
// ... 18 lines not shown
```

### lash_amd/csrc/sketch_kernels.hip

```cpp
#include "sketch_rules.h"

namespace lash {

template <int ALGO, int KMODE, bool XLOW, int REGS_, bool DIRECT, bool DEFER = false>
__global__ void __launch_bounds__(1024) LASH_SKETCH_WAVES_PER_EU_ATTR sketch_kernel(SketchArgs a)
{
    constexpr bool KEEP = REGS_ == REGS_LDS_KEEP;
    constexpr int REGS = KEEP ? REGS_LDS : REGS_;
    static_assert(!DEFER || (ALGO == 0 && REGS == REGS_LDS), "deferred signatures: HyperMinHash, one LDS table");
    static_assert(!KEEP || (!DIRECT && !DEFER && REGS == REGS_LDS), "keep bits: the packed launch with a plain LDS table");
    extern __shared__ __attribute__((aligned(16))) uint32_t lds_regs[];

    const uint32_t slot = xcd_skewed(blockIdx.x, gridDim.x);
    const uint32_t item = a.item_order ? a.item_order[slot] : slot + a.item_base;
    const WorkItem it = a.items[item];
#ifdef LASH_ITEM_TRACE_BUILD
    if (a.item_trace && threadIdx.x == 0) {
        uint32_t hw, xcc;
        asm volatile("s_getreg_b32 %0, hwreg(HW_REG_HW_ID)" : "=s"(hw));
        asm volatile("s_getreg_b32 %0, hwreg(HW_REG_XCC_ID)" : "=s"(xcc));
        a.item_trace[4ull * item] = wall_clock64();
        a.item_trace[4ull * item + 2] = ((unsigned long long)xcc << 32) | hw;
    }
#endif
    const GenomeDesc gd = a.genomes[it.genome];
    const uint64_t L = DIRECT ? gd.byte_len : a.nvalid[it.genome];
    const int k = a.k, p = a.p;
    const uint64_t nk = L >= (uint64_t)k ? L - (uint64_t)k + 1 : 0;
    const uint32_t nk_words = (uint32_t)((nk + 15) >> 4);
    const uint32_t fast_words = L >= 96 ? (uint32_t)((L - 96) >> 4) + 1u : 0u;
    if ((uint64_t)it.word_begin * 16 >= nk) {
        if ((it.slice & ITEM_SOLE) && !a.accumulate) {
            uint8_t *img = a.images + (uint64_t)it.genome * a.image_bytes;
            for (uint64_t i = threadIdx.x; i < a.image_bytes; i += blockDim.x) img[i] = 0;
            __syncthreads();
            if (threadIdx.x == 0) {
                const uint64_t n_regs = ALGO == 0 ? HMH_M : (1ull << p);
                write_header(img, a.lay.hdr_tpl, a.alpha_bits, n_regs, n_regs, (double)n_regs, ALGO == 0 ? HMH_P : p);
            }
        }
        return;
    }

    using Regs = SketchRegs<ALGO, REGS, XLOW, DEFER, true>;
    using SlowRegs = typename std::conditional<REGS == REGS_BYTES, LdsByteRegs, Regs>::type;
    Regs regs;
    uint32_t *census;
    bind_regs<ALGO, REGS>(a, it, item, lds_regs, regs, census);

    const uint32_t *__restrict__ w = a.words + gd.word_off;
    const bool multi_rec = gd.format != 0u || gd.rec_end - gd.rec_begin > 1;
    uint32_t RL = 0;
    if constexpr (DIRECT) {
        if (multi_rec && gd.format == 0u && a.nonuniform[it.genome] == 0u) RL = (uint32_t)(a.rec_off[gd.rec_begin + 1] - a.rec_off[gd.rec_begin]);
    }
    const bool use_bitmap = multi_rec && RL == 0u;
    const uint32_t *__restrict__ bk = use_bitmap ? (DIRECT ? a.brk_bytes : a.brk) + gd.brk_off : a.zero_words;
    const uint8_t *__restrict__ gseq = DIRECT ? a.seq + gd.byte_off : nullptr;
    uint32_t *const dirty = DIRECT ? a.dirty + it.genome : nullptr;
    KParams kp;
    kp.set_hashing<KMODE>(k, p, a.bitflip);
    const uint32_t cmask = a.lay.comp_mask;
    const CodeTabs ctabs{a.lay.code_lo, a.lay.code_hi};
    constexpr bool K21 = KMODE == KM_GT16 && DIRECT && !DEFER && (REGS == REGS_LDS || REGS == REGS_BYTES);
    uint32_t my_kmers = 0;
    const uint32_t lane = threadIdx.x & 63u;
    SigQueue sigq;
    sigq_init(sigq, (uint32_t)__builtin_amdgcn_readfirstlane((int)(a.stage_off + (threadIdx.x >> 6) * a.stage_stride)), a.sigq_depth, lane);
    if constexpr (Regs::QUEUED)
        regs.queue_init((uint32_t)__builtin_amdgcn_readfirstlane((int)(a.stage_off + (threadIdx.x >> 6) * a.stage_stride)), a.sigq_depth, lane);
    uint32_t tiles_dense = 0;
    bool judged = false;

    struct TileRegs { uint4 q; uint4 a1, a2, a3, la, lb; uint4 b; uint32_t c4, c5, dflag; };
    const uint32_t step = blockDim.x * SKETCH_WORDS_PER_THREAD;
    auto tile_active = [&](uint32_t tile) {
        const uint32_t w0 = tile + threadIdx.x * SKETCH_WORDS_PER_THREAD;
        return tile < it.word_end && w0 < it.word_end && w0 < nk_words;
    };
    const uint32_t w_last = it.word_end - SKETCH_WORDS_PER_THREAD;
    auto direct_fast = [&](uint32_t w0) { return w0 < fast_words; };
    auto tile_load = [&](uint32_t tile, TileRegs &t) {
        uint32_t w0 = tile + threadIdx.x * SKETCH_WORDS_PER_THREAD;
        w0 = w0 < w_last ? w0 : w_last;
        if constexpr (DIRECT) {
            const uint8_t *src = direct_fast(w0) ? gseq + (uint64_t)w0 * 16 : a.safe;
            t.q = load16_any(src); t.a1 = load16_any(src + 16); t.a2 = load16_any(src + 32); t.a3 = load16_any(src + 48);
            t.la = load16_any(src + 64);
            if constexpr (KMODE == KM_GT16) t.lb = load16_any(src + 80);
            t.dflag = __hip_atomic_load(dirty, __ATOMIC_RELAXED, __HIP_MEMORY_SCOPE_AGENT);
        } else {
            t.q = *reinterpret_cast<const uint4 *>(w + w0);
            t.c4 = w[w0 + 4];
            t.c5 = (KMODE == KM_GT16) ? w[w0 + 5] : 0u;
        }
        const uint32_t bi = use_bitmap ? w0 >> 1 : 0u;
        t.b = load16_any(reinterpret_cast<const uint8_t *>(bk + bi));
    };
    TileRegs nxt;
    tile_load(it.word_begin, nxt);
    if constexpr (REGS == REGS_LDS || REGS == REGS_BYTES) {
        for (uint32_t i = threadIdx.x; i < a.nreg32; i += blockDim.x) lds_regs[i] = ALGO == 2 ? 0u : RANK_EMPTY;
        asm volatile("s_waitcnt lgkmcnt(0)" ::: "memory");
    }
    __builtin_amdgcn_s_barrier();
    asm volatile("" ::: "memory");
#ifdef LASH_ABL_PROLOGUE_ONLY
    if (a.k != 99) return;
#endif
    for (uint32_t tile = it.word_begin; tile < it.word_end; tile += step) {
        const uint32_t w0 = tile + threadIdx.x * SKETCH_WORDS_PER_THREAD;
        const uint64_t pos0 = (uint64_t)w0 * 16;
        const bool active = tile_active(tile);
        const TileRegs cur = nxt;
        asm volatile("" ::"v"(cur.b.w));
        if (__builtin_amdgcn_ballot_w64(active) == 0ull) { tile_load(tile + step, nxt); continue; }

        const uint32_t junk = (threadIdx.x + 1u) * 0x9E3779B1u;
        uint32_t c0 = junk, c1 = ~junk, c2 = junk, c3 = ~junk, c4 = junk, c5 = ~junk;
        uint64_t kv = 0;
        if constexpr (DIRECT) {
            if (__builtin_expect(__builtin_amdgcn_readfirstlane((int)cur.dflag) != 0, 0)) break;
            uint32_t bad = 0;
            if (active) {
                if (__builtin_expect(direct_fast(w0), 1)) {
                    c0 = ascii16_to_word(cur.q, bad, ctabs); c1 = ascii16_to_word(cur.a1, bad, ctabs); c2 = ascii16_to_word(cur.a2, bad, ctabs);
                    c3 = ascii16_to_word(cur.a3, bad, ctabs); c4 = ascii16_to_word(cur.la, bad, ctabs);
                    if constexpr (KMODE == KM_GT16) c5 = ascii16_to_word(cur.lb, bad, ctabs);
                } else {
                    const TailWords t = ascii96_tail(gseq, (uint64_t)w0 * 16, L, ctabs);
                    c0 = t.w[0]; c1 = t.w[1]; c2 = t.w[2]; c3 = t.w[3]; c4 = t.w[4];
                    if constexpr (KMODE == KM_GT16) c5 = t.w[5];
                    bad |= t.bad;
                }
                if (RL) kv = uniform_valid_mask((uint32_t)pos0, RL, (uint32_t)nk, k);
                else kv = kmer_valid_mask(cur.b.x, cur.b.y, cur.b.z, (uint32_t)pos0, (uint32_t)nk, k);
            }
            if (__builtin_expect(__builtin_amdgcn_ballot_w64(bad != 0u) != 0ull, 0)) {
                const bool raw_ok = active && direct_fast(w0);
                {
                    const bool gone = raw_ok && (hopeless_bits(cur.q) & hopeless_bits(cur.a1) & hopeless_bits(cur.a2) & hopeless_bits(cur.a3) &
                                                 0x20202020u) == 0x20202020u;
                    const uint64_t act = __builtin_amdgcn_ballot_w64(active);
                    if (__builtin_amdgcn_ballot_w64(gone) == act) {
                        if ((threadIdx.x & 63) == 0) atomicAdd(a.ndel + it.genome, 64u * (uint32_t)__builtin_popcountll(act));
                        tile_load(tile + step, nxt);
                        continue;
                    }
                }
                tiles_dense = (uint32_t)__builtin_amdgcn_readfirstlane((int)tiles_dense) + 1u;
                if (tiles_dense >= 4u && tiles_dense * 8u > (tile - it.word_begin) / step + 1u && !judged) {
                    judged = true;
                    if ((threadIdx.x & 63) == 0 && atomicAdd(a.nslow + it.genome, 1u) + 1u >= gd.handover)
                        atomicOr(dirty, 1u);
                }
                bool dense = __builtin_popcountll(__builtin_amdgcn_ballot_w64(bad != 0u)) >= 16;
                uint32_t nd = 0, wave_nd = 0;
                uint64_t junc = 0, jstarts = 0;
                if (!dense) {
                    bool far = false;
                    if (active && bad != 0u) {
                        const InvMask im = lane_inv_mask(gseq, pos0, L);
                        const uint64_t W = window_or(im.lo, im.hi, k);
                        const uint64_t in_gen = L - pos0 >= 64 ? ~0ull : ((1ull << (L - pos0)) - 1ull);
                        junc = ~im.lo & W & in_gen;
                        jstarts = junc ? (~im.lo & in_gen & ~((1ull << __builtin_ctzll(junc)) - 1ull)) : 0ull;
                        kv &= ~W;
                        const uint64_t own = pos0 + 64 >= nk ? L - pos0 : 64;
                        nd = (uint32_t)__builtin_popcountll(im.lo & in_gen) +
                             (own > 64 ? (uint32_t)__builtin_popcount(im.hi & ((own >= 96 ? 0u : (1u << (own - 64))) - 1u)) : 0u);
                        if (junc) {
                            const uint32_t bl = 63u - (uint32_t)__builtin_clzll(junc);
                            const uint64_t in_gen_hi = L - pos0 >= 96 ? 0xFFFFFFFFull : (L - pos0 > 64 ? ((1ull << (L - pos0 - 64)) - 1ull) : 0ull);
                            const uint64_t after = bl == 63u ? 0ull : (~im.lo & in_gen) >> (bl + 1u);
                            far = (uint32_t)__builtin_popcountll(after) + (uint32_t)__builtin_popcountll(~(uint64_t)im.hi & in_gen_hi) < (uint32_t)k - 1u &&
                                  pos0 + 96 < L;
                        }
                    }
                    wave_nd = wave_sum(nd);
                    dense = wave_nd > 1024u || __builtin_amdgcn_ballot_w64(far) != 0ull;
                }
                if (dense) {
                    const uint64_t P0 = 16ull * (tile + (threadIdx.x & ~63u) * SKETCH_WORDS_PER_THREAD);
                    uint64_t E = P0 + 4096 < 16ull * it.word_end ? P0 + 4096 : 16ull * it.word_end;
                    E = E < L ? E : L;
                    const uint32_t stage_b = a.stage_off + (threadIdx.x >> 6) * a.stage_stride;
                    if constexpr (DEFER) sigq_drain<true>(regs, kp.bitflip, p, sigq);
                    if constexpr (Regs::QUEUED) regs.template drain<true>();
                    my_kmers += wave_sum(dense_tile<ALGO, KMODE, XLOW, SlowRegs>(regs, kp, gseq, L, P0, E, use_bitmap ? bk : nullptr, RL, k, cmask, ctabs,
                                                                            (uint32_t)__builtin_amdgcn_readfirstlane((int)stage_b), dirty,
                                                                            a.ndel + it.genome, raw_ok, cur.q, cur.a1, cur.a2, cur.a3));
                    tile_load(tile + step, nxt);
                    continue;
                }
                if (wave_nd && (threadIdx.x & 63) == 0) atomicAdd(a.ndel + it.genome, wave_nd);
                uint32_t walked = 0;
                if (junc)
                    walked = junction_walk<ALGO, XLOW, SlowRegs>(regs, gseq, L, pos0, junc, jstarts, use_bitmap ? bk : nullptr, RL, k, kp.bitflip, p,
                                                             cmask, ctabs, dirty);
                my_kmers += wave_sum(walked);
            }
        } else if (active) {
            c0 = cur.q.x; c1 = cur.q.y; c2 = cur.q.z; c3 = cur.q.w; c4 = cur.c4; c5 = cur.c5;
            kv = kmer_valid_mask(cur.b.x, cur.b.y, cur.b.z, (uint32_t)pos0, (uint32_t)nk, k);
            if constexpr (KEEP) {
                const uint32_t *kb = a.keep + gd.brk_off + (w0 >> 1);
                kv &= (uint64_t)kb[0] | ((uint64_t)kb[1] << 32);
            }
        }
        tile_load(tile + step, nxt);
        const bool all_valid = __builtin_amdgcn_ballot_w64(kv != ~0ull) == 0ull;
        if (all_valid) my_kmers += 4096u;
        else my_kmers += wave_sum((uint32_t)__builtin_popcountll(kv));

        uint32_t r0 = rcword(c0, cmask), r1 = rcword(c1, cmask), r2 = (KMODE == KM_GT16) ? rcword(c2, cmask) : 0u;
        if constexpr (REGS == REGS_BINS) regs.mode = 1u;
#pragma unroll LASH_WORD_UNROLL
        for (int wi = 0; wi < SKETCH_WORDS_PER_THREAD; ++wi) {
            hash_word<ALGO, KMODE, XLOW, Regs, K21 ? 21 : 0, DEFER>(regs, kp, c0, c1, c2, r0, r1, r2, all_valid, (uint32_t)kv, sigq, K21 && k == 21);
            if constexpr (REGS == REGS_BINS) {
                if (regs.overflowed()) {
                    regs.mode = 2u;
                    uint32_t kvw = (uint32_t)kv;
                    asm volatile("" : "+v"(kvw));
                    (void)process_word<ALGO, KMODE, XLOW, true, false>(regs, kp, c0, c1, c2, r0, r1, r2, kvw);
                    regs.mode = 1u;
                }
                if ((((uint32_t)wi + 1u) & (a.bin_flush_words - 1u)) == 0u) regs.flush(lane);
            }
            c0 = c1; c1 = c2; c2 = c3; c3 = c4; c4 = c5; c5 = 0;
            r0 = r1;
            if constexpr (KMODE == KM_GT16) { r1 = r2; r2 = rcword(c2, cmask); } else { r1 = rcword(c1, cmask); }
            kv >>= 16;
        }
        if constexpr (REGS == REGS_BINS) regs.mode = 0u;
    }

    if constexpr (DEFER) sigq_drain<true>(regs, kp.bitflip, p, sigq);
    if constexpr (Regs::QUEUED) regs.template drain<true>();
#ifdef LASH_ABL_NO_FLUSH
    if (a.k != 99) return;
#endif
    finish_item<ALGO, REGS, Regs>(a, it, regs, census, my_kmers, p, item);
#ifdef LASH_ITEM_TRACE_BUILD
    if (a.item_trace && threadIdx.x == 0) a.item_trace[4ull * item + 1] = wall_clock64();
#endif
}

constexpr uint32_t RING_W = 260, RING_BW = 130;
constexpr uint32_t STREAM_CHUNK = 2048, STREAM_BATCH = 2048;
static_assert(RING_W <= DENSE_STAGE_CODE_WORDS && RING_BW <= DENSE_STAGE_BRK_WORDS, "the ring lives in dense_tile's staging area");

template <int ALGO, int KMODE, bool XLOW, int REGS, bool DEFER = false>
__global__ void __launch_bounds__(1024) stream_sketch_kernel(SketchArgs a)
{
    static_assert(!DEFER || (ALGO == 0 && REGS == REGS_LDS), "deferred signatures: HyperMinHash, one LDS table");
    extern __shared__ __attribute__((aligned(16))) uint32_t lds_regs[];
    const uint32_t slot = xcd_skewed(blockIdx.x, gridDim.x);
    const uint32_t item = a.item_order ? a.item_order[slot] : slot + a.item_base;
    const WorkItem it = a.items[item];
    if (a.dirty[it.genome] == 0u) return;
    const GenomeDesc gd = a.genomes[it.genome];
    const uint64_t L = gd.byte_len;
    const int k = a.k, p = a.p;
    const uint64_t nkg = L >= (uint64_t)k ? L - (uint64_t)k + 1 : 0;
    if ((uint64_t)it.word_begin * 16 >= nkg) {
        write_empty_sole_image<ALGO>(a, it, p);
        return;
    }
    using Regs = SketchRegs<ALGO, REGS, XLOW, DEFER, false>;
    Regs regs;
    uint32_t *census;
    bind_regs<ALGO, REGS>(a, it, item, lds_regs, regs, census);
    if constexpr (REGS == REGS_LDS || REGS == REGS_BYTES) arm_table<ALGO>(a, lds_regs);
    const bool multi_rec = gd.rec_end - gd.rec_begin > 1;
    uint32_t RL = 0;
    if (multi_rec && a.nonuniform[it.genome] == 0u) RL = (uint32_t)(a.rec_off[gd.rec_begin + 1] - a.rec_off[gd.rec_begin]);
    const uint32_t *__restrict__ bk = (multi_rec && RL == 0u) ? a.brk_bytes + gd.brk_off : nullptr;
    const bool breaks = bk != nullptr || RL != 0u;
    const uint8_t *__restrict__ gseq = a.seq + gd.byte_off;
    KParams kp;
    kp.set_hashing<KMODE>(k, p, a.bitflip);
    const uint32_t cmask = a.lay.comp_mask;
    const CodeTabs ct{a.lay.code_lo, a.lay.code_hi};

    const uint32_t lane = threadIdx.x & 63u, wave = threadIdx.x >> 6, n_waves = blockDim.x >> 6;
    const uint32_t stage_b = (uint32_t)__builtin_amdgcn_readfirstlane((int)(a.stage_off + wave * (DENSE_STAGE_WORDS * 4u)));
    const uint32_t brk_b = stage_b + 4u * DENSE_STAGE_CODE_WORDS;
    lds_u32 *const ring = (lds_u32 *)(uintptr_t)stage_b;
    lds_u32 *const bring = (lds_u32 *)(uintptr_t)brk_b;
    SigQueue sigq;
    sigq_init(sigq, (uint32_t)__builtin_amdgcn_readfirstlane((int)(a.stage_off + n_waves * (DENSE_STAGE_WORDS * 4u) + wave * (64u * a.sigq_depth * 4u))),
              a.sigq_depth, lane);
    for (uint32_t i = lane; i < DENSE_STAGE_WORDS; i += 64u) ring[i] = 0;
    __syncthreads();

    const uint64_t B0 = 16ull * it.word_begin, B1 = 16ull * it.word_end < L ? 16ull * it.word_end : L;
    const uint64_t span = (((B1 - B0 + n_waves - 1) / n_waves) + STREAM_CHUNK - 1) & ~(uint64_t)(STREAM_CHUNK - 1);
    const uint64_t ws = B0 + (uint64_t)wave * span, we = ws + span < B1 ? ws + span : B1;
    uint32_t my_kmers = 0;
    if (ws < B1) {
        const uint32_t want = (uint32_t)k - 1u;
        uint32_t head_w = 0, have = 0, own_left = 0, la_have = 0, own_seen = 0;
        bool pend = false, stop = false;
        auto hash_batch = [&](uint32_t nstarts) {
            const uint32_t pos0 = 32u * lane;
            const bool active = pos0 < nstarts;
            const uint32_t junk = (threadIdx.x + 1u) * 0x9E3779B1u;
            uint32_t c0 = junk, c1 = ~junk, c2 = junk, c3 = ~junk, c4 = 0, c5 = 0;
            uint32_t kvw = 0;
            auto rw = [&](uint32_t j) { uint32_t w = head_w + 2u * lane + j; w = w >= RING_W ? w - RING_W : w; return w; };
            const uint32_t w0 = rw(0), w1 = rw(1);
            if (active) {
                c0 = ring[w0]; c1 = ring[w1]; c2 = ring[rw(2)]; c3 = ring[rw(3)];
                uint32_t b0 = 0, b1 = 0;
                if (breaks) {
                    uint32_t bw = (head_w >> 1) + lane; bw = bw >= RING_BW ? bw - RING_BW : bw;
                    const uint32_t bw1 = bw + 1u == RING_BW ? 0u : bw + 1u;
                    b0 = bring[bw]; b1 = bring[bw1];
                }
                kvw = (uint32_t)kmer_valid_mask(b0, b1, 0u, pos0, nstarts, k);
            }
            const bool all_valid = __builtin_amdgcn_ballot_w64(kvw != 0xFFFFFFFFu) == 0ull;
            my_kmers += all_valid ? 2048u : wave_sum((uint32_t)__builtin_popcount(kvw));
            __builtin_amdgcn_fence(__ATOMIC_ACQ_REL, "wavefront");
// ... 815 lines not shown
```

### lash_amd/csrc/sketch_rules.h

```cpp
#pragma once
#include <hip/hip_runtime.h>

#include <algorithm>
#include <cstdlib>
#include <type_traits>

#include "lash_device.h"
#include "lash_kernels.h"


constexpr uint32_t BINS_APPLY_RARE = 62;
#ifndef LASH_BINS_APPLY_LOADS
#define LASH_BINS_APPLY_LOADS 4
#endif
#ifndef LASH_WORD_UNROLL
#define LASH_WORD_UNROLL 1
#endif

namespace lash {

enum { KM_16 = 0, KM_LT16 = 1, KM_GT16 = 2 };

constexpr uint32_t RANK_EMPTY = 0xFFFFFFFFu;

// ... 175 lines not shown
    __device__ __forceinline__ void ull_add(uint32_t idx, uint32_t nlz) const
    {
        if ((nlz & 63u) == 63u) return;
        __attribute__((address_space(3))) uint32_t *w = (__attribute__((address_space(3))) uint32_t *)(uintptr_t)(idx & ~3u);
        const uint32_t sh = (idx & 3u) * 8u, single = 4u * ((nlz & 63u) + (uint32_t)p - 1u);
        uint32_t cur = *w;
        for (;;) {
            const uint32_t r = (cur >> sh) & 0xFFu, nr = ull_merge_fast(r, single);
            if (nr == r) break;
            const uint32_t want = (cur & ~(0xFFu << sh)) | (nr << sh);
            if (__hip_atomic_compare_exchange_strong(w, &cur, want, __ATOMIC_RELAXED, __ATOMIC_RELAXED, __HIP_MEMORY_SCOPE_WORKGROUP)) break;
        }
    }
    __device__ __forceinline__ uint32_t get_word(uint32_t i) const { return *(__attribute__((address_space(3))) uint32_t *)(uintptr_t)(i * 4u); }
    __device__ __forceinline__ uint32_t get(uint32_t) const { return 0u; }
    __device__ __forceinline__ void smax(uint32_t, uint32_t) const {}
    __device__ __forceinline__ void bor_first(uint32_t, int, uint32_t) const {}
    __device__ __forceinline__ void bor_pair(uint32_t, uint32_t, uint32_t) const {}
    static __device__ __forceinline__ void lds_wait() { asm volatile("s_waitcnt lgkmcnt(0)" ::: "memory"); }
};

template <int ALGO>
struct LdsByteQRegs : LdsByteRegs {
    static constexpr bool QUEUED = true;
    mutable uint32_t qptr;
    uint32_t q_lane_b, q_lim;
    static __device__ __forceinline__ uint32_t ld(uint32_t b) { return *(__attribute__((address_space(3))) uint32_t *)(uintptr_t)b; }
    static __device__ __forceinline__ void st(uint32_t b, uint32_t v) { *(__attribute__((address_space(3))) uint32_t *)(uintptr_t)b = v; }
    __device__ __forceinline__ void queue_init(uint32_t wave_base_b, uint32_t depth, uint32_t lane)
    {
        q_lane_b = wave_base_b + lane * depth * 4u;
        qptr = q_lane_b;
        q_lim = q_lane_b + 4u * (depth - 4u);
    }
    __device__ __forceinline__ void hll_max(uint32_t j, uint32_t raw) const
    {
        const int cur = *(__attribute__((address_space(3))) int8_t *)(uintptr_t)j;
        st(qptr, (j << 8) | (raw & 0xFFu));
        qptr += (int)raw > cur ? 4u : 0u;
    }
    __device__ __forceinline__ void ull_add(uint32_t idx, uint32_t nlz) const
    {
        const uint32_t r = *(__attribute__((address_space(3))) uint8_t *)(uintptr_t)idx;
        int ts = (int)(r - ((nlz << 2) + 4u * (uint32_t)p - 5u));
        asm("v_med3_i32 %0, %1, 0, 15" : "=v"(ts) : "v"(ts));
        st(qptr, (idx << 6) | (nlz & 63u));
        qptr += (0x2984u >> ts) & 4u;
    }
    template <bool ALL>
    __device__ __forceinline__ void drain() const
    {
        do {
            if (qptr != q_lane_b) {
                qptr -= 4u;
                const uint32_t e = ld(qptr);
                if constexpr (ALGO == 1) LdsByteRegs::hll_max(e >> 8, e & 0xFFu);
                else LdsByteRegs::ull_add(e >> 6, e & 63u);
            }
        } while (__builtin_amdgcn_ballot_w64(ALL ? qptr != q_lane_b : qptr > q_lim) != 0ull);
    }
    __device__ __forceinline__ void check() const { if (__builtin_amdgcn_ballot_w64(qptr > q_lim) != 0ull) drain<false>(); }
};

template <uint32_t CAP_>
struct LdsThrRegsT {
    uint32_t *base;
    static constexpr bool THR = true, BINS = false, BYTES = false, QUEUED = false;
    static constexpr uint32_t CAP = CAP_;
    static constexpr bool XLOW = CAP_ != 16u;
    static constexpr uint32_t REDO_BELOW = 1u << (31u - CAP_);
    static __device__ __forceinline__ uint32_t encode(uint32_t lzm1, uint32_t sig)
    {
        const uint32_t m = lzm1 < CAP ? lzm1 : CAP;
        return ((0xFFFFu >> m) << 16) | (0xFFFEu - (((lzm1 - m) << 10) | sig));
    }
    __device__ __forceinline__ void push_rank(uint32_t bucket, uint32_t lzm1, uint32_t sig, uint32_t vm) const
    { asm volatile("ds_min_u32 %0, %1" ::"v"(bucket << 2), "v"(encode(lzm1, sig) | ~vm) : "memory"); }
    __device__ __forceinline__ void push_rank_fast(uint32_t bucket, uint32_t lzm1, uint32_t sig, uint32_t vm) const
    {
        uint32_t thr = (0xFFFF0000u >> lzm1) & 0xFFFF0000u;
        if constexpr (CAP < 16u) thr |= (0xFFFF0000u >> CAP) & 0xFFFF0000u;
        asm volatile("ds_min_u32 %0, %1" ::"v"(bucket << 2), "v"((thr | (0xFFFEu - sig)) | ~vm) : "memory");
    }
    __device__ __forceinline__ uint32_t get(uint32_t i) const
    {
        const uint32_t w = base[i];
        if (w == 0xFFFFFFFFu) return RANK_EMPTY;
        const uint32_t thr = w >> 16, t = 0xFFFEu - (w & 0xFFFFu);
        const uint32_t m = thr ? (uint32_t)__builtin_clz(thr) - 16u : 16u;
        return ((m + (t >> 10)) << 10) | (t & 0x3FFu);
    }
    static __device__ __forceinline__ void lds_wait() { asm volatile("s_waitcnt lgkmcnt(0)" ::: "memory"); }
};
using LdsThrRegs = LdsThrRegsT<16u>;
using LdsThrRegsX = LdsThrRegsT<14u>;

enum { REGS_LDS = 0, REGS_GLOBAL = 1, REGS_BINS = 2, REGS_BYTES = 3,
       REGS_LDS_KEEP = 4 };

template <int ALGO, bool XLOW, bool MASKED, bool FAST, class Regs, bool VSH = false>
__device__ __forceinline__ uint32_t add_kmer(const Regs &regs, uint32_t c_lo, uint32_t c_hi, uint32_t vm,
                                             BitFlip bitflip, int p, uint32_t ull_sh28 = 0)
{
    constexpr bool HLL_HIGH = ALGO == 1 && XLOW;
    if constexpr (ALGO == 0) {
        (void)c_hi;
        if constexpr (FAST) {
            uint32_t xh, sig;
            if constexpr (XLOW) xxh3_128_4b_hmh_fast_xlow(c_lo, bitflip, xh, sig);
            else xxh3_128_4b_hmh_fast(c_lo, bitflip, xh, sig);
            const uint32_t t18 = (xh << 14) | 0x3FFFu;
            if constexpr (Regs::THR) {
                regs.push_rank_fast(xh >> 18, ffbh_u32(t18), sig, MASKED ? vm : 0xFFFFFFFFu);
            } else {
                uint32_t raw = (ffbh_u32(t18) << 10) | sig;
                if constexpr (MASKED) raw |= ~vm;
                regs.smax(xh >> 18, raw);
            }
            return t18;
        } else {
            uint64_t lo, hi;
            xxh3_128_4b(c_lo, bitflip, lo, hi);
            const uint64_t x = XLOW ? lo : hi, y = XLOW ? hi : lo;
            const uint32_t xh = (uint32_t)(x >> 32), xl = (uint32_t)x;
            const uint32_t bucket = xh >> 18;
            const uint32_t th = alignbit(xh, xl, 18);
            const uint32_t tl = (xl << 14) | 0x3FFFu;
            const uint32_t lzm1 = clz64_nz(th, tl);
            if constexpr (Regs::THR) {
                regs.push_rank(bucket, lzm1, (uint32_t)y & 0x3FFu, MASKED ? vm : 0xFFFFFFFFu);
            } else {
                uint32_t raw = (lzm1 << 10) | ((uint32_t)y & 0x3FFu);
                if constexpr (MASKED) raw |= ~vm;
                regs.smax(bucket, raw);
            }
            return th;
        }
    } else if constexpr (ALGO == 1) {
        const uint32_t pm = (1u << p) - 1u;
        if constexpr (FAST && !HLL_HIGH) {
            const uint64_t g = xxh3_64_8b_pre(c_lo, c_hi, bitflip);
            const uint32_t gh = (uint32_t)(g >> 32), gl = (uint32_t)g;
            const uint32_t j = (gl ^ alignbit(gh, gl, 28)) & pm;
            uint32_t raw = ffbh_u32(gh);
            if constexpr (MASKED) raw |= ~vm;
            if constexpr (Regs::BINS) regs.push(j, raw);
            else if constexpr (Regs::BYTES) regs.hll_max(j, raw);
            else regs.smax(j, raw);
            return gh;
        }
        if constexpr (FAST && HLL_HIGH) {
            const uint64_t g = xxh3_64_8b_pre(c_lo, c_hi, bitflip);
            const uint32_t gh = (uint32_t)(g >> 32), gl = (uint32_t)g;
            const uint32_t t28 = gh >> (VSH ? ull_sh28 : (uint32_t)(28 - p));
            const uint32_t th = alignbit(gh, gl, 32 - p) ^ t28;
            uint32_t raw = ffbh_u32(th);
            if constexpr (MASKED) raw |= ~vm;
            const uint32_t jh = gh >> (32 - p);
            if constexpr (Regs::BINS) regs.push(jh, raw);
            else if constexpr (Regs::BYTES) regs.hll_max(jh, raw);
            else regs.smax(jh, raw);
            return th;
        }
        const uint64_t h = xxh3_64_8b(c_lo, c_hi, bitflip);
        const uint32_t hh = (uint32_t)(h >> 32), hl = (uint32_t)h;
        if constexpr (HLL_HIGH) {
            const uint32_t jh = hh >> (32 - p);
            uint32_t raw = clz64_nz(alignbit(hh, hl, 32 - p), (hl << p) | (1u << (p - 1)));
            if constexpr (MASKED) raw |= ~vm;
            if constexpr (Regs::BINS) regs.push(jh, raw);
// ... 930 lines not shown

template <int ALGO>
__device__ __forceinline__ BinRegs bin_regs_of(const SketchArgs &a, uint32_t genome)
{
    BinRegs r;
    const uint32_t wave = threadIdx.x >> 6, lane = threadIdx.x & 63u;
    r.sub_shift = a.bin_sub_shift;
    r.V = a.bins << r.sub_shift;
    r.sub_lane = lane & ((1u << r.sub_shift) - 1u);
    r.cnt_b = a.bin_lds_off + wave * a.bin_wave_bytes;
    r.stage_b = r.cnt_b + r.V * 4u;
    r.S = a.bin_S; r.RS = bin_row_stride(a.bin_S); r.bin_shift = a.bin_shift; r.algo = ALGO;
    r.mode = 0u; r.ovf = 0u;

    const uint32_t gi = genome - a.bin_genome0;
    const BinGenome bg = a.bin_genomes[gi];
    r.cap = bg.cap;
    r.lists = a.bin_lists + bg.list_off;
    r.cnt = a.bin_cnt + (uint64_t)gi * a.bins;
    r.slab = a.bin_slab + (uint64_t)gi * a.bin_slab_words;
    r.spill = a.bin_spill + (uint64_t)gi * a.bins;
    for (uint32_t b = lane; b < r.V; b += 64u) *(__attribute__((address_space(3))) uint32_t *)(uintptr_t)(r.cnt_b + b * 4u) = 0u;
    asm volatile("s_waitcnt lgkmcnt(0)" ::: "memory");
    return r;
}

template <class Kern>
inline hipError_t allow_dyn_lds(Kern kern, uint32_t lds)
{
    if (lds <= 48u * 1024u) return hipSuccess;
    return hipFuncSetAttribute(reinterpret_cast<const void *>(kern), hipFuncAttributeMaxDynamicSharedMemorySize, (int)lds);
}
template <class Kern, class Args>
inline hipError_t launch_dyn_lds(Kern kern, dim3 grid, dim3 threads, uint32_t lds, hipStream_t stream, const Args &args)
{
    const hipError_t e = allow_dyn_lds(kern, lds);
    if (e != hipSuccess) return e;
    hipLaunchKernelGGL(kern, grid, threads, lds, stream, args);
    return hipGetLastError();
}

template <int ALGO, int REGS, bool XLOW, bool DEFER, bool QUEUED>
using SketchRegs = typename std::conditional<DEFER, typename std::conditional<XLOW, LdsThrRegsX, LdsThrRegs>::type,
                            typename std::conditional<REGS == REGS_LDS, LdsRegs,
                            typename std::conditional<REGS == REGS_GLOBAL, GlobalRegs,
                            typename std::conditional<REGS == REGS_BINS, BinRegs,
                            typename std::conditional<QUEUED, LdsByteQRegs<ALGO>, LdsByteRegs>::type>::type>::type>::type>::type;

template <int ALGO, int REGS, class Regs>
__device__ __forceinline__ void bind_regs(const SketchArgs &a, const WorkItem &it, uint32_t item, uint32_t *lds_regs, Regs &regs, uint32_t *&census)
{
    if constexpr (REGS == REGS_BINS) {
        regs = bin_regs_of<ALGO>(a, it.genome);
        census = lds_regs;
    } else if constexpr (REGS == REGS_GLOBAL) {
        regs.base = a.gregs + (uint64_t)(item - a.item_base) * a.nreg32;
        census = lds_regs;
    } else {
        if ((uint32_t)(uintptr_t)(__attribute__((address_space(3))) uint32_t *)lds_regs != 0u) __builtin_trap();
        if constexpr (REGS == REGS_BYTES) regs.p = a.p;
        else regs.base = lds_regs;
        census = lds_regs + a.nreg32;
    }
}
template <int ALGO>
__device__ __forceinline__ void arm_table(const SketchArgs &a, uint32_t *lds_regs)
{
    for (uint32_t i = threadIdx.x; i < a.nreg32; i += blockDim.x) lds_regs[i] = ALGO == 2 ? 0u : RANK_EMPTY;
}
template <int ALGO>
__device__ __forceinline__ void write_empty_sole_image(const SketchArgs &a, const WorkItem it, int p)
{
    if ((it.slice & ITEM_SOLE) && !a.accumulate) {
        uint8_t *img = a.images + (uint64_t)it.genome * a.image_bytes;
        for (uint64_t i = threadIdx.x; i < a.image_bytes; i += blockDim.x) img[i] = 0;
        __syncthreads();
        if (threadIdx.x == 0) {
            const uint64_t n_regs = ALGO == 0 ? HMH_M : (1ull << p);
            write_header(img, a.lay.hdr_tpl, a.alpha_bits, n_regs, n_regs, (double)n_regs, ALGO == 0 ? HMH_P : p);
        }
    }
}

template <int ALGO, int REGS, class Regs>
__device__ __forceinline__ void finish_item(const SketchArgs &a, const WorkItem &it, const Regs &regs, uint32_t *census, uint32_t my_kmers, int p,
                                            uint32_t item)
{
    constexpr bool USE_LDS = REGS != REGS_GLOBAL;
    Regs::lds_wait();
    if ((threadIdx.x & 63) == 0) census[threadIdx.x >> 6] = my_kmers;
    if constexpr (!USE_LDS) __threadfence();
    __syncthreads();
    if (threadIdx.x == 0) {
        unsigned long long tot = 0;
        for (uint32_t i = 0; i < (blockDim.x >> 6); ++i) tot += census[i];
        a.item_kmers[item] = (uint32_t)tot;
    }

    if constexpr (REGS == REGS_BINS) {
        regs.finish(threadIdx.x & 63u);
        return;
    }
    const bool sole = (it.slice & ITEM_SOLE) != 0u;
    uint32_t *out = reinterpret_cast<uint32_t *>(a.partials + (uint64_t)item * a.partial_stride);
    uint8_t *img = a.images + (uint64_t)it.genome * a.image_bytes;
    const uint32_t HDR = a.lay.hdr_bytes, reg_be = ALGO == 0 ? a.lay.hmh_reg_be : 0u;
    uint32_t *hist = census + 16;
    if constexpr (ALGO == 1) {
        if (sole) {
            if (threadIdx.x < 72) hist[threadIdx.x] = 0;
            __syncthreads();
        }
    }
    HllTally tally;
    auto put = [&](uint32_t i, uint32_t v) {
        if (!sole) { out[i] = v; return; }
        uint8_t *dst = img + HDR + 4ull * i;
        if (a.accumulate) v = merge_word<ALGO>(hmh_img_order(load_u32_any(dst), reg_be), v);
        store_u32_any(dst, hmh_img_order(v, reg_be));
        if constexpr (ALGO == 1) tally.add(hist, v);
    };
    auto hmh_reg = [](uint32_t raw) { return (int32_t)raw < 0 ? 0u : raw + 0x400u; };
    auto hll_reg = [](uint32_t raw) { return raw + 1u; };
    if constexpr (REGS == REGS_BYTES) {
        for (uint32_t i = threadIdx.x; i < ((1u << p) >> 2); i += blockDim.x) {
            uint32_t w = regs.get_word(i);
            if constexpr (ALGO == 1) w = ((w & 0x7F7F7F7Fu) + 0x01010101u) ^ (w & 0x80808080u);
            put(i, w);
        }
        if constexpr (ALGO == 1) {
            if (sole) {
                tally.flush(hist);
                __syncthreads();
                if (threadIdx.x < 64u) write_hll_header_wave(img, a.lay.hdr_tpl, hist, a.alpha_bits, p, a.hll_corner ? a.hll_corner + it.genome : nullptr);
            }
        } else {
            if (sole && threadIdx.x == 0) write_header(img, a.lay.hdr_tpl, a.alpha_bits, 1ull << p, 0, 0.0, p);
        }
        return;
    }
    if constexpr (ALGO == 0) {
        for (uint32_t i = threadIdx.x; i < HMH_M / 2; i += blockDim.x)
            put(i, hmh_reg(regs.get(2 * i)) | (hmh_reg(regs.get(2 * i + 1)) << 16));
        if (sole && threadIdx.x == 0 && HDR) write_header(img, a.lay.hdr_tpl, a.alpha_bits, HMH_M, 0, 0.0, HMH_P);
    } else if constexpr (ALGO == 1) {
        const uint32_t nw = (1u << p) >> 2;
        for (uint32_t i = threadIdx.x; i < nw; i += blockDim.x)
            put(i, hll_reg(regs.get(4 * i)) | (hll_reg(regs.get(4 * i + 1)) << 8) | (hll_reg(regs.get(4 * i + 2)) << 16) | (hll_reg(regs.get(4 * i + 3)) << 24));
        if (sole) {
            tally.flush(hist);
            __syncthreads();
            if (threadIdx.x < 64u) write_hll_header_wave(img, a.lay.hdr_tpl, hist, a.alpha_bits, p, a.hll_corner ? a.hll_corner + it.genome : nullptr);
        }
    } else {
        const uint32_t nw = (1u << p) >> 2;
        for (uint32_t i = threadIdx.x; i < nw; i += blockDim.x) {
            uint32_t o = 0;
#pragma unroll
            for (int b = 0; b < 4; ++b) {
                const uint32_t lo = regs.get(8 * i + 2 * b), hi = regs.get(8 * i + 2 * b + 1);
                uint32_t r = 0;
                if (lo | hi) {
                    const uint64_t x = (((uint64_t)hi << 32) | lo) << (p - 1);
                    const uint32_t top = 63u - (uint32_t)__builtin_clzll(x);
                    const uint32_t below = top >= 2 ? (uint32_t)(x >> (top - 2)) & 3u : (uint32_t)(x << (2 - top)) & 3u;
                    r = (top << 2) | below;
// ... 11 lines not shown
```

Measured before the change: 1277 billion k-mers/s.

## Seed HMH registers with a rank floor and redo genomes that leave buckets empty

For deferred HMH sole items, the register table now starts at a floor rank derived from the expected k-mers per bucket, so LDS min-updates below the floor become no-ops. If any register is still at the floor after the pass, the item is flagged and a second redo launch recomputes that genome with no floor. A host probe tracks the redo fraction and switches the floor off when redos become common. The cost is an extra register scan and vote per item, an always-issued redo launch that mostly exits early, and some added bookkeeping.

```diff
diff --git a/include/lash_gfx950.h b/include/lash_gfx950.h
--- a/include/lash_gfx950.h
+++ b/include/lash_gfx950.h
@@ -70,6 +70,7 @@
     float    direct_ms;
     uint32_t defer_launches;
     uint32_t sole_launches;
+    uint32_t floor_redone;
 } lash_timing;
 
 int         lash_abi_version(void);
diff --git a/lash_amd/_lib.py b/lash_amd/_lib.py
--- a/lash_amd/_lib.py
+++ b/lash_amd/_lib.py
@@ -27,7 +27,8 @@
     _fields_ = [("pack_ms", C.c_float), ("sketch_ms", C.c_float), ("finalize_ms", C.c_float), ("calls", C.c_uint32),
                 ("sketch_launches", C.c_uint32), ("sketch_workgroups", C.c_uint32), ("direct_launches", C.c_uint32),
                 ("kmers", C.c_uint64), ("bases_last", C.c_uint64), ("packed_bytes", C.c_uint64),
-                ("direct_ms", C.c_float), ("defer_launches", C.c_uint32), ("sole_launches", C.c_uint32)]
+                ("direct_ms", C.c_float), ("defer_launches", C.c_uint32), ("sole_launches", C.c_uint32),
+                ("floor_redone", C.c_uint32)]
 
 
 class ClusterStats(C.Structure):
diff --git a/lash_amd/csrc/lash_api.hip b/lash_amd/csrc/lash_api.hip
--- a/lash_amd/csrc/lash_api.hip
+++ b/lash_amd/csrc/lash_api.hip
@@ -236,7 +236,7 @@
     release(ctx->sole_state);
     for (DevBuf *b : {&ctx->items, &ctx->item_begin, &ctx->item_kmers, &ctx->partials, &ctx->gregs, &ctx->counter, &ctx->st_seq, &ctx->st_rec,
                       &ctx->st_img, &ctx->hll_flags, &ctx->ec_ref, &ctx->ec_qry, &ctx->ec_x, &ctx->ec_card, &ctx->wf_scratch, &ctx->wf_out, &ctx->top_buf,
-                      &ctx->fa_off, &ctx->fa_scratch, &ctx->fc_scratch, &ctx->kf_keep})
+                      &ctx->fa_off, &ctx->fa_scratch, &ctx->fc_scratch, &ctx->kf_keep, &ctx->floor_flags})
         release(*b);
     {
         lash_packed &sc = ctx->scratch;
@@ -358,6 +358,9 @@
         unsigned long long c = 0;
         HIPCHK(ctx, hipMemcpy(&c, ctx->counter.ptr, 8, hipMemcpyDeviceToHost));
         t.kmers = c;
+        uint32_t redone = 0;
+        HIPCHK(ctx, hipMemcpy(&redone, static_cast<const uint8_t *>(ctx->counter.ptr) + 64, 4, hipMemcpyDeviceToHost));
+        t.floor_redone = redone;
     }
     if (ctx->last_sole_only && ctx->counter.ptr && ctx->counter_zeroed) {
         unsigned long long b = 0;
@@ -455,10 +458,7 @@
     TraceScope trace_scope(ctx->trace);
     TRACE("call");
     static const bool env_no_direct = getenv("LASH_NO_DIRECT") != nullptr;
-    if (ctx->probe_pending && hipEventQuery(ctx->probe_ev) == hipSuccess) {
-        ctx->dirty_frac = ctx->probe_tiles ? (float)ctx->probe_host[0] / (float)ctx->probe_tiles : 0.f;
-        ctx->probe_pending = false;
-    }
+    probe_collect(ctx);
     bool direct = !(prm->flags & LASH_F_NO_DIRECT) && !env_no_direct;
     bool stream_first = false;
     if (direct && ctx->dirty_frac > 0.2f) {
diff --git a/lash_amd/csrc/lash_common.h b/lash_amd/csrc/lash_common.h
--- a/lash_amd/csrc/lash_common.h
+++ b/lash_amd/csrc/lash_common.h
@@ -24,6 +24,7 @@
 };
 
 constexpr uint32_t ITEM_SOLE        = 0x8000u;
+constexpr uint32_t ITEM_Z0_SHIFT    = 16;
 constexpr int      PAD_WORDS        = 8;
 constexpr int      SKETCH_WORDS_PER_THREAD = 4;
 constexpr int      HMH_P            = 14;
diff --git a/lash_amd/csrc/lash_ctx.h b/lash_amd/csrc/lash_ctx.h
--- a/lash_amd/csrc/lash_ctx.h
+++ b/lash_amd/csrc/lash_ctx.h
@@ -176,6 +176,7 @@
     DevBuf ec_ref, ec_qry, ec_x, ec_card;
     DevBuf wf_scratch, wf_out;
     DevBuf top_buf;
+    DevBuf floor_flags;
     DevBuf hll_flags;
     uint32_t hll_flags_n = 0;
     bool hll_flags_on_host = false;
@@ -189,6 +190,10 @@
     uint32_t probe_tiles = 0;
     float dirty_frac = 0.f;
     uint32_t direct_skipped = 0;
+    bool probe_dirty_valid = false;
+    uint32_t probe_floor_items = 0;
+    float floor_frac = 0.f;
+    uint32_t floor_skipped = 0;
 };
 
 namespace {
diff --git a/lash_amd/csrc/lash_hll_replay.hip b/lash_amd/csrc/lash_hll_replay.hip
--- a/lash_amd/csrc/lash_hll_replay.hip
+++ b/lash_amd/csrc/lash_hll_replay.hip
@@ -30,11 +30,14 @@
 struct ReplayRestore {
     lash_ctx *c;
     lash_timing last; bool timing; std::vector<const lash_packed *> packed; float dirty_frac; uint32_t direct_skipped; bool sole_only;
+    float floor_frac; uint32_t floor_skipped;
     explicit ReplayRestore(lash_ctx *x) : c(x), last(x->last), timing(x->timing), packed(x->last_packed), dirty_frac(x->dirty_frac),
-                                          direct_skipped(x->direct_skipped), sole_only(x->last_sole_only) {}
+                                          direct_skipped(x->direct_skipped), sole_only(x->last_sole_only), floor_frac(x->floor_frac),
+                                          floor_skipped(x->floor_skipped) {}
     ~ReplayRestore()
     {
         c->last = last; c->timing = timing; c->last_packed = packed; c->dirty_frac = dirty_frac; c->direct_skipped = direct_skipped;
+        c->floor_frac = floor_frac; c->floor_skipped = floor_skipped;
         c->last_sole_only = sole_only;
         c->probe_pending = false;
     }
diff --git a/lash_amd/csrc/lash_internal.h b/lash_amd/csrc/lash_internal.h
--- a/lash_amd/csrc/lash_internal.h
+++ b/lash_amd/csrc/lash_internal.h
@@ -10,7 +10,8 @@
 int pack_into(lash_ctx *ctx, lash_packed *pk, hipStream_t stream, EvSet *ev, const uint8_t *d_seq, const uint8_t *d_seq_end,
               const uint64_t *d_rec_off, uint64_t n_rec, const uint64_t *genome_rec_off, const uint64_t *genome_byte_off,
               uint32_t n_genomes, const uint8_t *formats = nullptr, bool direct = false);
-int probe_dirty(lash_ctx *ctx, lash_packed *pk, hipStream_t stream);
+int probe_post(lash_ctx *ctx, lash_packed *pk, const uint32_t *d_floor_call, uint32_t floor_items, hipStream_t stream);
+void probe_collect(lash_ctx *ctx);
 uint64_t sole_max_bytes(const lash_ctx *ctx, const lash_params *prm, const SolePlan &sp);
 int sole_run(lash_ctx *ctx, const lash_params *prm, const SolePlan &sp, uint64_t max_len, const uint8_t *d_seq, uint64_t seq_bytes,
              const uint64_t *d_rec_off, uint64_t n_rec, bool any_multi, bool rec_identity, const uint64_t *genome_byte_off, const lash_packed *pk,
diff --git a/lash_amd/csrc/lash_kernels.h b/lash_amd/csrc/lash_kernels.h
--- a/lash_amd/csrc/lash_kernels.h
+++ b/lash_amd/csrc/lash_kernels.h
@@ -56,6 +56,9 @@
     uint32_t          bin_lds_off, bin_wave_bytes;
     uint32_t          bin_slab_words;
     uint32_t          bin_genome0;
+    uint32_t         *floor_flags;
+    uint32_t         *floor_count;
+    uint32_t          floor_redo;
 };
 
 struct SketchPlan {
diff --git a/lash_amd/csrc/lash_plan.hip b/lash_amd/csrc/lash_plan.hip
--- a/lash_amd/csrc/lash_plan.hip
+++ b/lash_amd/csrc/lash_plan.hip
@@ -151,22 +151,34 @@
     return LASH_OK;
 }
 
-int probe_dirty(lash_ctx *ctx, lash_packed *pk, hipStream_t stream)
-{
-    uint32_t *tbc = static_cast<uint32_t *>(pk->tile_begin_c.ptr);
-    HIPCHK(ctx, launch_dirty_tile_scan(pk->d_tile_begin, pk->d_dirty, pk->n_genomes, tbc, tbc + pk->n_genomes + 1, stream));
+int probe_post(lash_ctx *ctx, lash_packed *pk, const uint32_t *d_floor_call, uint32_t floor_items, hipStream_t stream)
+{
+    uint32_t *tbc = pk ? static_cast<uint32_t *>(pk->tile_begin_c.ptr) : nullptr;
+    if (pk) HIPCHK(ctx, launch_dirty_tile_scan(pk->d_tile_begin, pk->d_dirty, pk->n_genomes, tbc, tbc + pk->n_genomes + 1, stream));
+    if (!pk && !floor_items) return LASH_OK;
     if (!ctx->probe_host) {
         HIPCHK(ctx, hipHostMalloc(reinterpret_cast<void **>(&ctx->probe_host), 64, hipHostMallocDefault));
-        ctx->probe_host[0] = 0;
+        ctx->probe_host[0] = ctx->probe_host[1] = 0;
         HIPCHK(ctx, hipEventCreateWithFlags(&ctx->probe_ev, hipEventDisableTiming));
     }
     if (!ctx->probe_pending) {
-        HIPCHK(ctx, hipMemcpyAsync(ctx->probe_host, tbc + pk->n_genomes + 1, 4, hipMemcpyDeviceToHost, stream));
+        if (pk) HIPCHK(ctx, hipMemcpyAsync(ctx->probe_host, tbc + pk->n_genomes + 1, 4, hipMemcpyDeviceToHost, stream));
+        if (floor_items) HIPCHK(ctx, hipMemcpyAsync(ctx->probe_host + 1, d_floor_call, 4, hipMemcpyDeviceToHost, stream));
         HIPCHK(ctx, hipEventRecord(ctx->probe_ev, stream));
         ctx->probe_pending = true;
-        ctx->probe_tiles = pk->h_tile_begin.empty() ? 0 : pk->h_tile_begin.back();
-    }
-    return LASH_OK;
+        ctx->probe_dirty_valid = pk != nullptr;
+        ctx->probe_tiles = !pk || pk->h_tile_begin.empty() ? 0 : pk->h_tile_begin.back();
+        ctx->probe_floor_items = floor_items;
+    }
+    return LASH_OK;
+}
+
+void probe_collect(lash_ctx *ctx)
+{
+    if (!ctx->probe_pending || hipEventQuery(ctx->probe_ev) != hipSuccess) return;
+    if (ctx->probe_dirty_valid) ctx->dirty_frac = ctx->probe_tiles ? (float)ctx->probe_host[0] / (float)ctx->probe_tiles : 0.f;
+    if (ctx->probe_floor_items) ctx->floor_frac = (float)ctx->probe_host[1] / (float)ctx->probe_floor_items;
+    ctx->probe_pending = false;
 }
 
 uint64_t bins_budget_bytes(lash_ctx *ctx)
@@ -491,15 +503,32 @@
     uint32_t tail_split;
     bool tail_geo;
     int64_t defer_min;
+    int floor_margin;
+    int floor_force;
 };
+
+#ifndef LASH_HMH_FLOOR_MARGIN
+#define LASH_HMH_FLOOR_MARGIN 5
+#endif
+static uint32_t floor_z0(uint64_t n_kmers, uint32_t cap, const PlanKnobs &knobs)
+{
+    if (knobs.floor_margin < 0) return 0u;
+    if (knobs.floor_force >= 0) return std::min<uint32_t>((uint32_t)knobs.floor_force, cap);
+    const uint64_t per_bucket = n_kmers / HMH_M;
+    if (per_bucket == 0) return 0u;
+    const int z0 = 63 - __builtin_clzll(per_bucket) - knobs.floor_margin;
+    return z0 > 0 ? std::min<uint32_t>((uint32_t)z0, cap) : 0u;
+}
+
 static PlanKnobs plan_knobs()
 {
     static const uint64_t slice_factor = getenv("LASH_SLICE_FACTOR") ? std::max(1, atoi(getenv("LASH_SLICE_FACTOR"))) : 0;
     static const uint64_t item_cap = getenv("LASH_ITEM_CAP_WORDS") ? std::max(1024, atoi(getenv("LASH_ITEM_CAP_WORDS"))) : 0;
     static const uint32_t tail_split = getenv("LASH_TAIL_SPLIT") ? (uint32_t)std::max(1, atoi(getenv("LASH_TAIL_SPLIT"))) : 0u;
     const char *dm_env = getenv("LASH_DEFER_MIN");
+    const char *fm_env = getenv("LASH_HMH_FLOOR_MARGIN"), *fz_env = getenv("LASH_HMH_FLOOR_Z0");
     return PlanKnobs{slice_factor, item_cap, tail_split, !(getenv("LASH_TAIL_GEO") && atoi(getenv("LASH_TAIL_GEO")) == 0),
-                     dm_env ? atoll(dm_env) : 600000};
+                     dm_env ? atoll(dm_env) : 600000, fm_env ? atoi(fm_env) : LASH_HMH_FLOOR_MARGIN, fz_env ? atoi(fz_env) : -1};
 }
 
 static bool may_defer(const SketchPlan &plan) { return plan.algo == LASH_HMH && plan.use_lds; }
@@ -514,10 +543,11 @@
     uint64_t n_coarse = 0;
     uint64_t total_words = 0;
     bool defer = false;
+    uint32_t n_floor = 0;
 };
 
 static ItemPlan plan_items(const std::vector<uint64_t> &blen, const SketchPlan &plan, uint64_t slots, bool direct, bool stream_first,
-                           const PlanKnobs &knobs)
+                           const PlanKnobs &knobs, const std::vector<uint64_t> *floor_kmers = nullptr)
 {
     const uint32_t n_genomes = (uint32_t)blen.size();
     const bool defer_eligible = may_defer(plan);
@@ -606,6 +636,13 @@
         for (uint32_t i = 0; i < n_items; ++i) ip.order[count[bucket(ip.items[i].word_end - ip.items[i].word_begin)]++] = i;
     }
     ip.defer = defer_eligible && ip.n_coarse > 0 && knobs.defer_min >= 0 && ip.total_words * 16 / ip.n_coarse >= (uint64_t)knobs.defer_min;
+    if (ip.defer && floor_kmers && !(direct && stream_first))
+        for (WorkItem &w : ip.items) {
+            if (!(w.slice & ITEM_SOLE)) continue;
+            const uint32_t z0 = floor_z0((*floor_kmers)[w.genome], plan.variant ? 14u : 16u, knobs);
+            w.slice |= z0 << ITEM_Z0_SHIFT;
+            ip.n_floor += z0 != 0u;
+        }
     return ip;
 }
 
@@ -717,6 +754,12 @@
     bool identity = pk->n_rec == n;
     for (uint32_t g = 0; g < n && identity; ++g) identity = pk->h_descs[g].rec_begin == g && pk->h_descs[g].rec_end == g + 1u;
     return sole_run(ctx, prm, sp, sole_max, pk->d_seq, gbo[n], pk->d_rec_off, pk->n_rec, pk->any_multi, identity, gbo.data(), nullptr, n, images, ndel);
+}
+
+static SketchArgs floor_redo_args(SketchArgs a)
+{
+    a.floor_redo = 1u;
+    return a;
 }
 
 static int direct_launches(lash_ctx *ctx, const lash_params *prm, const SketchPlan &plan, lash_packed *pk, const ItemPlan &ip, SketchArgs &sa,
@@ -739,6 +782,7 @@
     if (timed) HIPCHK(ctx, hipEventRecord(ev->e[6], ctx->stream));
     rc = launch_items(ctx, plan, prm, sa, br, ip.item_begin, d_item_begin, [&](const SketchArgs &a, uint32_t cnt) -> int {
         if (direct_pass) HIPCHK(ctx, launch_sketch(plan, a, cnt, ctx->stream, true));
+        if (direct_pass && ip.n_floor) HIPCHK(ctx, launch_sketch(plan, floor_redo_args(a), cnt, ctx->stream, true));
         if (ranged) HIPCHK(ctx, launch_sketch_stream(plan, a, cnt, ctx->stream));
         return LASH_OK;
     });
@@ -746,7 +790,7 @@
     if (timed) { HIPCHK(ctx, hipEventRecord(ev->e[5], ctx->stream)); ev->direct = true; }
     if ((rc = item_trace_end(ctx, ip, plan.threads, sa))) return rc;
     if (direct_pass) {
-        if ((rc = probe_dirty(ctx, pk, ctx->stream))) return rc;
+        if ((rc = probe_post(ctx, pk, ip.n_floor ? sa.floor_count + 1 : nullptr, ip.n_floor, ctx->stream))) return rc;
         ctx->last.direct_launches += n_items ? 1 : 0;
         ctx->last.defer_launches += (n_items && plan.defer) ? 1 : 0;
     }
@@ -785,7 +829,14 @@
     const uint32_t lds_wg = plan.lds_bytes + ((pk->direct || may_defer(plan) || plan.bytes) ? sketch_direct_stage_bytes(plan) : 0u);
     const uint32_t wg_per_cu = plan.use_lds ? std::max(1u, (160u * 1024u) / std::max(lds_wg, 1u)) : 4u;
     const uint64_t slots = (uint64_t)ctx->cu_count * std::min(wg_per_cu, 2048u / plan.threads);
-    const ItemPlan ip = plan_items(blen, plan, slots, pk->direct, pk->stream_first, plan_knobs());
+    std::vector<uint64_t> floor_kmers(n_genomes, 0);
+    for (uint32_t g = 0; g < n_genomes && pk->h_descs.size() == n_genomes; ++g) {
+        const GenomeDesc &d = pk->h_descs[g];
+        const uint64_t recs = d.format == 0u && d.rec_end > d.rec_begin ? d.rec_end - d.rec_begin : 1;
+        const uint64_t bases = d.format == 2u ? blen[g] / 2 : blen[g], lost = recs * (uint64_t)(prm->k - 1);
+        floor_kmers[g] = bases > lost ? bases - lost : 0;
+    }
+    ItemPlan ip = plan_items(blen, plan, slots, pk->direct, pk->stream_first, plan_knobs(), d_keep ? nullptr : &floor_kmers);
     const uint32_t n_items = (uint32_t)ip.items.size();
     plan.defer = ip.defer && !d_keep;
     if (d_keep && !sketch_plan_keeps(plan)) return LASH_EINVAL;
@@ -802,6 +853,13 @@
     BinsRun br;
     if ((rc = reserve_stage(ctx, prm, plan, ip, entries, br))) return rc;
     if (!br.fits) return sketch_from(ctx, prm, pk, d_out_images, ev, false, d_keep);
+    probe_collect(ctx);
+    if (ip.n_floor && ctx->floor_frac > 0.2f) {
+        if (++ctx->floor_skipped < 8) {
+            for (WorkItem &w : ip.items) w.slice &= (1u << ITEM_Z0_SHIFT) - 1u;
+            ip.n_floor = 0;
+        } else ctx->floor_skipped = 0;
+    }
     const WorkItem *d_items;
     const uint32_t *d_item_begin, *d_item_order = nullptr;
     {
@@ -851,15 +909,24 @@
     sa.nvalid = pk->d_nvalid;
     sa.item_order = d_item_order;
     sa.safe = static_cast<const uint8_t *>(ctx->counter.ptr) + 128;
+    if (ip.n_floor) {
+        if ((rc = reserve(ctx, ctx->floor_flags, (size_t)n_genomes * 4))) return rc;
+        HIPCHK(ctx, hipMemsetAsync(ctx->floor_flags.ptr, 0, (size_t)n_genomes * 4, ctx->stream));
+        sa.floor_flags = static_cast<uint32_t *>(ctx->floor_flags.ptr);
+        sa.floor_count = reinterpret_cast<uint32_t *>(static_cast<uint8_t *>(ctx->counter.ptr) + 64);
+        HIPCHK(ctx, hipMemsetAsync(sa.floor_count + 1, 0, 4, ctx->stream));
+    }
     if (d_keep) sa.keep = d_keep;
     if (pk->direct) {
         if ((rc = direct_launches(ctx, prm, plan, mpk, ip, sa, br, d_item_begin, ev))) return rc;
     } else {
         rc = launch_items(ctx, plan, prm, sa, br, ip.item_begin, d_item_begin, [&](const SketchArgs &a, uint32_t cnt) -> int {
             HIPCHK(ctx, d_keep ? launch_sketch_keep(plan, a, cnt, ctx->stream) : launch_sketch(plan, a, cnt, ctx->stream));
+            if (ip.n_floor) HIPCHK(ctx, launch_sketch(plan, floor_redo_args(a), cnt, ctx->stream));
             return LASH_OK;
         });
         if (rc) return rc;
+        if (ip.n_floor && (rc = probe_post(ctx, nullptr, sa.floor_count + 1, ip.n_floor, ctx->stream))) return rc;
         ctx->last.defer_launches += (n_items && plan.defer) ? 1 : 0;
     }
     if (n_sole && (rc = sole_batch(ctx, prm, sole_plan, sole_max, pk, d_out_images, pk->stream_first ? sa.ndel2 : sa.ndel))) return rc;
diff --git a/lash_amd/csrc/sketch_kernels.hip b/lash_amd/csrc/sketch_kernels.hip
--- a/lash_amd/csrc/sketch_kernels.hip
+++ b/lash_amd/csrc/sketch_kernels.hip
@@ -14,6 +14,9 @@
     const uint32_t slot = xcd_skewed(blockIdx.x, gridDim.x);
     const uint32_t item = a.item_order ? a.item_order[slot] : slot + a.item_base;
     const WorkItem it = a.items[item];
+    if constexpr (DEFER) {
+        if (a.floor_redo && a.floor_flags[it.genome] == 0u) return;
+    }
 #ifdef LASH_ITEM_TRACE_BUILD
     if (a.item_trace && threadIdx.x == 0) {
         uint32_t hw, xcc;
@@ -100,7 +103,8 @@
     TileRegs nxt;
     tile_load(it.word_begin, nxt);
     if constexpr (REGS == REGS_LDS || REGS == REGS_BYTES) {
-        for (uint32_t i = threadIdx.x; i < a.nreg32; i += blockDim.x) lds_regs[i] = ALGO == 2 ? 0u : RANK_EMPTY;
+        const uint32_t empty = ALGO == 2 ? 0u : (DEFER ? LdsThrRegs::floor_word(item_z0(a, it)) : RANK_EMPTY);
+        for (uint32_t i = threadIdx.x; i < a.nreg32; i += blockDim.x) lds_regs[i] = empty;
         asm volatile("s_waitcnt lgkmcnt(0)" ::: "memory");
     }
     __builtin_amdgcn_s_barrier();
@@ -241,6 +245,9 @@
 #ifdef LASH_ABL_NO_FLUSH
     if (a.k != 99) return;
 #endif
+    if constexpr (DEFER) {
+        if (floor_left(a, it, lds_regs, dirty)) return;
+    }
     finish_item<ALGO, REGS, Regs>(a, it, regs, census, my_kmers, p, item);
 #ifdef LASH_ITEM_TRACE_BUILD
     if (a.item_trace && threadIdx.x == 0) a.item_trace[4ull * item + 1] = wall_clock64();
diff --git a/lash_amd/csrc/sketch_rules.h b/lash_amd/csrc/sketch_rules.h
--- a/lash_amd/csrc/sketch_rules.h
+++ b/lash_amd/csrc/sketch_rules.h
@@ -281,10 +281,12 @@
         if constexpr (CAP < 16u) thr |= (0xFFFF0000u >> CAP) & 0xFFFF0000u;
         asm volatile("ds_min_u32 %0, %1" ::"v"(bucket << 2), "v"((thr | (0xFFFEu - sig)) | ~vm) : "memory");
     }
+    static __host__ __device__ constexpr uint32_t floor_word(uint32_t z0) { return ((0xFFFFu >> z0) << 16) | 0xFFFFu; }
+    static __device__ __forceinline__ bool is_floor(uint32_t w) { return (w & 0xFFFFu) == 0xFFFFu; }
     __device__ __forceinline__ uint32_t get(uint32_t i) const
     {
         const uint32_t w = base[i];
-        if (w == 0xFFFFFFFFu) return RANK_EMPTY;
+        if (is_floor(w)) return RANK_EMPTY;
         const uint32_t thr = w >> 16, t = 0xFFFEu - (w & 0xFFFFu);
         const uint32_t m = thr ? (uint32_t)__builtin_clz(thr) - 16u : 16u;
         return ((m + (t >> 10)) << 10) | (t & 0x3FFu);
@@ -1381,6 +1383,35 @@
     }
 }
 
+__device__ __forceinline__ uint32_t item_z0(const SketchArgs &a, const WorkItem &it) { return a.floor_redo ? 0u : (it.slice >> ITEM_Z0_SHIFT) & 31u; }
+__device__ __forceinline__ bool floor_left(const SketchArgs &a, const WorkItem &it, uint32_t *lds_regs, uint32_t *dirty)
+{
+    if (item_z0(a, it) == 0u) return false;
+    asm volatile("s_waitcnt lgkmcnt(0)" ::: "memory");
+    __syncthreads();
+    bool left = false;
+    for (uint32_t i = threadIdx.x; i < HMH_M; i += blockDim.x) left = left || (lds_regs[i] & 0xFFFFu) == 0xFFFFu;
+    uint32_t *vote = lds_regs + a.nreg32;
+    const uint32_t wave_left = __builtin_amdgcn_ballot_w64(left) != 0ull;
+    if ((threadIdx.x & 63u) == 0u) vote[threadIdx.x >> 6] = wave_left;
+    __syncthreads();
+    uint32_t any = 0;
+    for (uint32_t wv = 0; wv < (blockDim.x >> 6); ++wv) any |= vote[wv];
+    __syncthreads();
+    if (!any) return false;
+    if (dirty && __hip_atomic_load(dirty, __ATOMIC_RELAXED, __HIP_MEMORY_SCOPE_AGENT) != 0u) return true;
+    if (threadIdx.x == 0) {
+        a.floor_flags[it.genome] = 1u;
+        atomicAdd(a.floor_count, 1u);
+        atomicAdd(a.floor_count + 1, 1u);
+        if (dirty) {
+            atomicExch(a.ndel + it.genome, 0u);
+            atomicExch(a.nslow + it.genome, 0u);
+        }
+    }
+    return true;
+}
+
 template <int ALGO, int REGS, class Regs>
 __device__ __forceinline__ void finish_item(const SketchArgs &a, const WorkItem &it, const Regs &regs, uint32_t *census, uint32_t my_kmers, int p,
                                             uint32_t item)
```

Result: no change. 1283 billion k-mers/s, median of 4 (+0.4%).
